# MiraPurkrabek/ProbPose_code

Hardware: AMD Instinct MI355X
Metric: person-crops/sec @ 256x192 bs64 (higher is better)
Workload: dtype f16x3; 1 GPU; ProbPose-small (ViT-S 12x384, 12 heads x 32) bs64 random 256x192 uint8 crops per GPU, flip_test=True, seeded random-init weights: preprocess -> backbone x2 passes -> ProbMapHead (heatmap branch + Sparsemax + 4 towers) -> ProbMap decode -> results in pinned host memory; crops_per_gpu=64, global_batch=64, parallelism=dp1, steps_in_flight=2

## Files before the change

### include/probpose_mi355x.h

```cpp
#ifndef PROBPOSE_MI355X_H_
#define PROBPOSE_MI355X_H_

#include <stddef.h>
#include <stdint.h>

#ifdef __cplusplus
extern "C" {
#endif

#define PP_ABI_VERSION 4


enum {
    PP_OK = 0,
    PP_ERR_INVALID_ARG = -1,
    PP_ERR_UNSUPPORTED = -2,
    PP_ERR_HIP = -3,
    PP_ERR_WORKSPACE = -4
};

#define PP_MAX_RADIUS 9
#define PP_MAX_TAPS (2 * PP_MAX_RADIUS + 1)

int pp_abi_version(void);
const char* pp_last_error(void);
const char* pp_status_string(int status);

int pp_device_cu_count(void);

int pp_stream_create(void** stream_out);
int pp_stream_destroy(void* stream);

int pp_set_option(const char* name, int value);
int pp_get_option(const char* name, int* value);

long long pp_launch_count(const char* kernel);
int pp_reset_launch_counts(void);

typedef struct {
    int prec, n_img, n_tokens, embed, ffn, patch_k, n_keypoints, feat_h, feat_w, heat_h, heat_w, deconv_channels;
} pp_plan_shape;
enum {
    PP_WS_PATCHES = 0,
    PP_WS_X = 1,
    PP_WS_H = 2,
    PP_WS_QKV = 3,
    PP_WS_ATT = 4,
    PP_WS_LN2 = 5,
    PP_WS_FFN = 6,
    PP_WS_FEAT = 7,
    PP_WS_LOGITS = 8,
    PP_WS_DECONV = 9,
    PP_WS_TOWER = 10,
    PP_WS_TOWER_PARTIAL = 11,
    PP_WS_TOWER_POOLED = 12,
    PP_WS_WINOGRAD = 13,
    PP_WS_LN_STATS = 14
};
long long pp_workspace_bytes(int buffer, int index, const pp_plan_shape* shape);

int pp_conv3x3_splitk_slices(int prec, int B, int H, int W, int Cin, int Cout, int groups);

int pp_clock_probe(unsigned long long* out_cycles_ticks, const unsigned long long* stop_flag, unsigned int max_microseconds, void* stream);

int pp_probmap_decode(const float* hm, const float* hm_flip, const int32_t* flip_indices,
                      const double* taps, const int32_t* radius,
                      int B, int K, int H, int W, double in_w, double in_h,
                      float* avg_out, float* conv_out,
                      float* locs, double* keypoints, float* scores, void* stream);

int pp_probmap_head_decode(const float* logits, const float* logits_flip, const int32_t* flip_indices,
                           const double* taps, const int32_t* radius,
                           int B, int K, int H, int W, double in_w, double in_h,
                           float temperature, float normalize,
                           float* avg_out, float* conv_out,
                           float* locs, double* keypoints, float* scores, void* stream);

enum { PP_PREC_BF16 = 0, PP_PREC_F32 = 1, PP_PREC_F16X3 = 2 };
enum { PP_OUT_F32 = 0, PP_OUT_BF16 = 1, PP_OUT_SPLIT = 2 };
enum { PP_ACT_NONE = 0, PP_ACT_GELU = 1, PP_ACT_RELU = 2 };
enum { PP_CONV3X3 = 1, PP_DECONV4X4S2 = 2 };

int pp_gemm(int prec, const void* act, const void* weight, const float* bias, const float* residual,
            int res_mod, void* out, int M, int N, int K, int lda, int ldw, int ldc, int act_fn,
            int out_bf16, int planar_P, void* stream);
int pp_gemm_ws(int prec, const void* act, const void* weight, const float* bias, const float* residual,
               int res_mod, void* out, int M, int N, int K, int lda, int ldw, int ldc, int act_fn,
               int out_bf16, int planar_P, float w_inv_scale, void* stream);

int pp_linear_ln_folded(const void* act, const void* weight, const float* bias, const void* residual, int residual_format,
                        void* out, int out_format, int M, int N, int K, int act_fn, const float* ln_stats,
                        const float* ln_colsum, float ln_eps, float* stats_out, void* stream);
int pp_linear_ln_folded_ws(const void* act, const void* weight, const float* bias, const void* residual, int residual_format,
                           void* out, int out_format, int M, int N, int K, int act_fn, const float* ln_stats,
                           const float* ln_colsum, float ln_eps, float* stats_out, float w_inv_scale, void* stream);
int pp_linear_ln_folded_supported(int M, int N, int K, int with_ln_stats);

int pp_skinny_linear(const void* act, const void* weight, const float* bias, const float* residual, int res_mod, void* out, int out_format,
                     int M, int N, int K, int act_fn, float w_inv_scale, const float* ln_gamma, const float* ln_beta, float ln_eps,
                     void* ln_out, int* ln_counters, void* stream);
int pp_skinny_linear_tile(int M, int N, int K, int with_layernorm);
int pp_skinny_conv1x1_planar(const void* act, const void* weight_padded, const float* bias_padded, float* out, int n_img, int P, int K,
                             int n_valid, float w_inv_scale, void* stream);
int pp_skinny_deconv(const void* act_nhwc, const void* weight, const float* bias, void* out_nhwc, int B, int H, int W, int Cin, int Cout,
                     void* stream);

int pp_gemm_residual_layernorm(int prec, const void* act, const void* weight, const float* bias,
                               const float* residual, int res_mod, float* x_out, const float* gamma,
                               const float* beta, float eps, void* h_out, int h_bf16, int M, int N, int K,
                               int lda, int ldw, void* stream);
int pp_gemm_residual_layernorm_ws(int prec, const void* act, const void* weight, const float* bias,
                               const float* residual, int res_mod, float* x_out, const float* gamma,
                               const float* beta, float eps, void* h_out, int h_bf16, int M, int N, int K,
                               int lda, int ldw, float w_inv_scale, void* stream);

int pp_mlp_residual_layernorm(const void* h_in, const void* w1, const float* b1, const void* w2,
                              const float* b2, const float* residual, float* x_out, const float* gamma,
                              const float* beta, float eps, void* h_out, int M, int E, int F, void* stream);

int pp_proj_mlp_residual_layernorm(const void* attn, const void* wp, const float* bp, const float* residual,
                                   const float* gamma2, const float* beta2, const void* w1, const float* b1,
                                   const void* w2, const float* b2, float* x_out, const float* gamma,
                                   const float* beta, float eps, void* h_out, const void* wqkv, const float* bqkv,
                                   void* qkv_out, int M, int E, int F, void* stream);

int pp_conv_gemm(int prec, int kind, const void* act_nhwc, const void* weight, const float* bias, void* out,
                 int B, int H, int W, int Cin, int Cout, int py, int px, int groups,
                 long long stride_act_g, long long stride_w_g, long long stride_out_g,
                 long long stride_bias_g, int ldc, int act_fn, int out_bf16, void* stream);

int pp_attention(int prec, const void* qkv, void* out, int n_seq, int seq_len, int heads, int head_dim,
                 float scale, void* stream);

int pp_preproc_im2col(int prec, const void* img, int img_is_f32, void* patches, int B, int passes, int H,
                      int W, int patch, int pad, const float* mean_host, const float* std_host,
                      int bgr_to_rgb, void* stream);

int pp_layernorm(const float* x, const float* gamma, const float* beta, void* y, int M, int E, float eps,
                 int out_bf16, void* stream);

int pp_maxpool_relu_nhwc(const void* in, int in_bf16, void* out, int out_bf16, int N, int H, int W, int C,
                         int ph, int pw, void* stream);

int pp_conv3x3_maxpool_relu(int prec, const void* act_nhwc, const void* weight, const float* bias, void* out_pooled,
                            void* scratch_full, int B, int H, int W, int Cin, int Cout, int ph, int pw, int groups,
                            long long stride_act_g, long long stride_w_g, long long stride_bias_g, int fmt, void* stream);

int pp_vit_layer(const void* qkv_in, int seq_len, int heads, float scale, const void* wp, const float* bp,
                 const float* residual, const float* gamma2, const float* beta2, const void* w1, const float* b1,
                 const void* w2, const float* b2, float* x_out, const float* gamma, const float* beta, float eps,
                 void* h_out, const void* wqkv, const float* bqkv, void* qkv_out, int M, int E, int F, void* stream);

long long pp_ffn_split_packed_bytes(int E, int F);
int pp_ffn_split_pack_weights(const void* w1_split, const void* w2_split, void* packed, int E, int F, void* stream);
int pp_ffn_split_residual_layernorm(const void* h_in, const void* w_packed, const float* b1, const float* b2,
                                    const float* residual, float* x_out, const float* gamma, const float* beta,
                                    float eps, void* h_out, int M, int E, int F, void* stream);
int pp_ffn_split_residual_layernorm_ws(const void* h_in, const void* w_packed, const float* b1, const float* b2,
                                       const float* residual, float* x_out, const float* gamma, const float* beta,
                                       float eps, void* h_out, int M, int E, int F, float w1_inv_scale, float w2_inv_scale, void* stream);

int pp_qkv_attention_split(const void* h_in, const void* wqkv, const float* bqkv, void* out, int n_seq, int seq_len, int heads,
                           int head_dim, float scale, void* stream);
int pp_qkv_attention_split_ws(const void* h_in, const void* wqkv, const float* bqkv, void* out, int n_seq, int seq_len, int heads,
                              int head_dim, float scale, float w_inv_scale, void* stream);

int pp_qkv_attention_split_folded(const void* x_centered, const void* wqkv_folded, const float* bqkv_folded, const float* ln_stats, void* out,
                                  int n_seq, int seq_len, int heads, int head_dim, float scale, float w_inv_scale, void* stream);

long long pp_proj_split_packed_bytes(int E);
int pp_proj_split_pack_weights(const void* wp_split, void* packed, int E, void* stream);
int pp_proj_ffn_split_residual_layernorm(const void* att, const void* wproj_packed, const float* bproj,
                                         const float* gamma2, const float* beta2, void* h_scratch, const void* w_packed,
                                         const float* b1, const float* b2, const float* residual, float* x_out,
                                         const float* gamma, const float* beta, float eps, void* h_out, int M, int E,
                                         int F, void* stream);
int pp_proj_ffn_split_residual_layernorm_ws(const void* att, const void* wproj_packed, const float* bproj,
                                            const float* gamma2, const float* beta2, void* h_scratch, const void* w_packed,
                                            const float* b1, const float* b2, const float* residual, float* x_out,
                                            const float* gamma, const float* beta, float eps, void* h_out, int M, int E,
                                            int F, float wp_inv_scale, float w1_inv_scale, float w2_inv_scale, void* stream);

int pp_proj_ffn_split_folded(const void* att, const void* wproj_packed, const float* bproj, const float* gamma2, const float* beta2,
                             void* h_scratch, const void* w_packed, const float* b1, const float* b2, const void* residual,
                             int residual_format, const float* residual_stats, int fold_out, float* x_out, const float* gamma,
                             const float* beta, float eps, void* h_out, float* stats_out, int M, int E, int F, float wp_inv_scale,
                             float w1_inv_scale, float w2_inv_scale, void* stream);

int pp_deconv_head(const void* act_nhwc, const void* weight, const float* bias, const void* head_w, const float* head_b,
                   float* logits_phased, int B, int H, int W, int Cin, int Cout, int K, void* stream);

int pp_deconv_head_split(const void* act_nhwc, const void* weight, const float* bias, const void* head_w_packed,
                         const float* head_b, float* logits_phased, int B, int H, int W, int Cin, int Cout, int K, void* stream);

int pp_probmap_head_decode_phased(const float* logits, const float* logits_flip, const int32_t* flip_indices,
                                  const double* taps, const int32_t* radius, int B, int K, int H, int W, double in_w,
                                  double in_h, float temperature, float normalize, float* avg_out, float* conv_out,
                                  float* locs, double* keypoints, float* scores, void* stream);

#define PP_DECODE_LOGITS 1
#define PP_DECODE_PHASED 2
#define PP_DECODE_SHIFT_HEATMAP 4
int pp_probmap_decode_flags(const float* maps, const float* maps_flip, const int32_t* flip_indices, const double* taps,
                            const int32_t* radius, int B, int K, int H, int W, double in_w, double in_h, float temperature,
                            float normalize, float* avg_out, float* conv_out, float* locs, double* keypoints, float* scores,
                            int flags, void* stream);

int pp_udp_heatmap_decode(const float* maps, const float* maps_flip, const int32_t* flip_indices, int B, int K, int H, int W,
                          double in_w, double in_h, int blur_kernel_size, float* avg_out, float* locs, double* keypoints,
                          float* scores, int flags, void* stream);

int pp_conv3x3_splitk(int prec, const void* act_nhwc, const void* weight, float* partials, int B, int H, int W, int Cin,
                      int Cout, int groups, long long stride_act_g, long long stride_w_g, int ksplit, void* stream);
int pp_sum_maxpool_relu_nhwc(const float* partials, int nsplit, long long split_stride, const float* bias,
                             int images_per_group, void* out, int out_bf16, int N, int H, int W, int C, int ph, int pw,
                             void* stream);

long long pp_winograd_scratch_bytes(int B, int H, int W, int Cin);
int pp_conv3x3_winograd_maxpool_relu(const void* act_nhwc, const void* u_packed, const float* bias, void* v_scratch,
                                     void* out_pooled, int B, int H, int W, int Cin, int Cout, int pool_h, int pool_w, int groups,
                                     void* stream);

int pp_tower_final(const void* feat, int feat_bf16, const float* w, const float* bias,
                   const int32_t* flip_indices, float* out, int B, int passes, int C, int K, float err_div,
                   void* stream);

int pp_extended_oks(const double* gt_kpts, const double* gt_bbox, const double* gt_area, const double* dt_kpts,
                    const double* sigmas, const int* gt_visibilities, int G, int D, int K, int n_vis,
                    double confidence_thr, double padding, int use_area, int original, double* out, void* stream);

int pp_pack_records(const double* keypoints, const float* scores, const float* scalars, double* records, int n, void* stream);

int pp_revert_heatmaps_max(const float* heatmaps, const double* inverse_maps, float* out, int n, int K, int hm_h, int hm_w,
                           int img_h, int img_w, void* stream);

int pp_heatmap_posterior(float* heatmaps, const float* presence, double* scratch, int K, int H, int W, void* stream);

int pp_exoks_cells(const double* gt_kpts, const double* gt_bbox, const double* gt_area, const double* dt_kpts,
                   const double* sigmas, const int* gt_visibilities, const int* cell_gt_off, const int* cell_dt_off,
                   const long long* cell_out_off, int n_cells, int K, int n_vis, double confidence_thr, double padding,
                   int use_area, int original, double* out, void* stream);

int pp_exoks_match(const double* ious, const int* cell_gt_off, const int* cell_dt_off, const long long* cell_iou_off,
                   const unsigned char* gt_ignore, const unsigned char* gt_iscrowd, const double* gt_area,
                   const double* gt_bbox, const double* dt_area, const double* dt_bbox, const double* area_rng,
                   const double* iou_thrs, int n_cells, int max_gt_per_cell, int N_gt, int N_dt, int L, int A, int T,
                   int match_by_bbox, int* dt_match, unsigned char* dt_ignore, int* gt_match,
                   unsigned char* gt_ignore_out, double* sim_sum, int* sim_cnt, void* stream);

int pp_exmap_accumulate(const int* dt_match, const unsigned char* dt_ignore, const unsigned char* gt_ignore,
                        const int* order, const double* dt_score, const double* rec_thrs, int n_cells, int N_gt, int N_dt,
                        int L, int A, int T, int R, int* chunk_scratch, double* precision, double* recall, double* scores,
                        void* stream);

int pp_warp_affine_u8(const void* img_hwc, int img_h, int img_w, int channels, const double* inverse_maps, void* crops_chw,
                      int n, int out_h, int out_w, void* stream);
int pp_warp_affine_u8_batch(const void* const* images, const int* image_hw, int channels, const int* crop_image,
                            const double* inverse_maps, int max_img_h, int max_img_w, void* crops_chw, int n, int out_h,
                            int out_w, void* stream);

long long pp_parea_scratch_bytes(int K, int H, int W);
int pp_parea_thresholds(const float* maps, int K, int H, int W, void* scratch, float* thr, int* draw, void* stream);
int pp_parea_compose(const void* image_rgb, int img_h, int img_w, int pad_left, int pad_top, const float* maps, int K,
                     const float* thr, const int* draw, const int* boxes, int n_boxes, void* canvas_rgb, int canvas_h,
                     int canvas_w, void* stream);
int pp_draw_poses(const void* image_rgb, int img_h, int img_w, const float* keypoints, const float* visible, const int* boxes,
                  int n, int K, const int* skeleton, const void* link_rgb, const void* kpt_rgb, int n_links, double kpt_thr,
                  float radius, float thickness, float alpha, void* out_rgb, void* stream);
int pp_resize_bilinear_u8(const void* src_rgb, int src_h, int src_w, void* dst_rgb, int dst_h, int dst_w, void* stream);

#ifdef __cplusplus
}
#endif
#endif
```

### probpose_code_amd/_lib.py

```python
import ctypes
import os
from ctypes import c_char_p, c_double, c_float, c_int, c_longlong, c_void_p

import torch

_HERE = os.path.dirname(os.path.abspath(__file__))
LIB_NAME = "libprobpose_mi355x.so"
LIB_PATH = os.path.join(_HERE, LIB_NAME)

PP_OK = 0
PP_ERR_INVALID_ARG = -1
PP_ERR_UNSUPPORTED = -2
PP_ERR_HIP = -3
PP_ERR_WORKSPACE = -4
PP_MAX_RADIUS = 9
PP_MAX_TAPS = 2 * PP_MAX_RADIUS + 1


class ProbPoseLibraryError(RuntimeError):

    def __init__(self, fn, status, message):
        super().__init__(f"{fn} failed with {status}: {message}")
        self.status = status


def _load():
    if not os.path.exists(LIB_PATH):
        raise ImportError(
            f"{LIB_PATH} not found. Build it first: `python -c 'import __graft_entry__ as g; g.build()'` "
            "or `make -C probpose_code_amd/csrc`. There is no CPU fallback for the ProbPose hot path."
        )
    return ctypes.CDLL(LIB_PATH)


lib = _load()

_P = c_void_p
SIGNATURES = {
    "pp_abi_version": (c_int, []),
    "pp_last_error": (c_char_p, []),
    "pp_status_string": (c_char_p, [c_int]),
    "pp_device_cu_count": (c_int, []),
    "pp_stream_create": (c_int, [_P]),
    "pp_stream_destroy": (c_int, [_P]),
    "pp_set_option": (c_int, [c_char_p, c_int]),
    "pp_get_option": (c_int, [c_char_p, _P]),
    "pp_launch_count": (c_longlong, [c_char_p]),
    "pp_reset_launch_counts": (c_int, []),
    "pp_workspace_bytes": (c_longlong, [c_int, c_int, _P]),
    "pp_conv3x3_splitk_slices": (c_int, [c_int] * 7),
    "pp_linear_ln_folded": (c_int, [_P, _P, _P, _P, c_int, _P, c_int, c_int, c_int, c_int, c_int, _P, _P, c_float, _P, _P]),
    "pp_linear_ln_folded_ws": (c_int, [_P, _P, _P, _P, c_int, _P, c_int, c_int, c_int, c_int, c_int, _P, _P, c_float, _P, c_float, _P]),
    "pp_linear_ln_folded_supported": (c_int, [c_int] * 4),
    "pp_skinny_linear": (c_int, [_P, _P, _P, _P, c_int, _P, c_int, c_int, c_int, c_int, c_int, c_float, _P, _P, c_float, _P, _P, _P]),
    "pp_skinny_linear_tile": (c_int, [c_int, c_int, c_int, c_int]),
    "pp_skinny_deconv": (c_int, [_P, _P, _P, _P, c_int, c_int, c_int, c_int, c_int, _P]),
    "pp_skinny_conv1x1_planar": (c_int, [_P, _P, _P, _P, c_int, c_int, c_int, c_int, c_float, _P]),
    "pp_clock_probe": (c_int, [_P, _P, ctypes.c_uint, _P]),
    "pp_probmap_decode": (
        c_int,
        [_P, _P, _P, _P, _P, c_int, c_int, c_int, c_int, c_double, c_double, _P, _P, _P, _P, _P, _P],
    ),
    "pp_probmap_head_decode": (
        c_int,
        [_P, _P, _P, _P, _P, c_int, c_int, c_int, c_int, c_double, c_double, c_float, c_float, _P, _P, _P, _P, _P, _P],
    ),
    "pp_probmap_head_decode_phased": (
        c_int,
        [_P, _P, _P, _P, _P, c_int, c_int, c_int, c_int, c_double, c_double, c_float, c_float, _P, _P, _P, _P, _P, _P],
    ),
    "pp_probmap_decode_flags": (
        c_int,
        [_P, _P, _P, _P, _P, c_int, c_int, c_int, c_int, c_double, c_double, c_float, c_float, _P, _P, _P, _P, _P, c_int, _P],
    ),
    "pp_udp_heatmap_decode": (
        c_int, [_P, _P, _P, c_int, c_int, c_int, c_int, c_double, c_double, c_int, _P, _P, _P, _P, c_int, _P]),
    "pp_deconv_head": (c_int, [_P, _P, _P, _P, _P, _P, c_int, c_int, c_int, c_int, c_int, c_int, _P]),
    "pp_deconv_head_split": (c_int, [_P, _P, _P, _P, _P, _P, c_int, c_int, c_int, c_int, c_int, c_int, _P]),
    "pp_gemm": (
        c_int,
        [c_int, _P, _P, _P, _P, c_int, _P, c_int, c_int, c_int, c_int, c_int, c_int, c_int, c_int, c_int, _P],
    ),
    "pp_gemm_ws": (
        c_int,
        [c_int, _P, _P, _P, _P, c_int, _P, c_int, c_int, c_int, c_int, c_int, c_int, c_int, c_int, c_int, c_float, _P],
    ),
    "pp_gemm_residual_layernorm": (
        c_int,
        [c_int, _P, _P, _P, _P, c_int, _P, _P, _P, c_float, _P, c_int, c_int, c_int, c_int, c_int, c_int, _P],
    ),
    "pp_gemm_residual_layernorm_ws": (
        c_int,
        [c_int, _P, _P, _P, _P, c_int, _P, _P, _P, c_float, _P, c_int, c_int, c_int, c_int, c_int, c_int, c_float, _P],
    ),
    "pp_mlp_residual_layernorm": (c_int, [_P, _P, _P, _P, _P, _P, _P, _P, _P, c_float, _P, c_int, c_int, c_int, _P]),
    "pp_proj_mlp_residual_layernorm": (
        c_int, [_P, _P, _P, _P, _P, _P, _P, _P, _P, _P, _P, _P, _P, c_float, _P, _P, _P, _P, c_int, c_int, c_int, _P]),
    "pp_vit_layer": (
        c_int, [_P, c_int, c_int, c_float, _P, _P, _P, _P, _P, _P, _P, _P, _P, _P, _P, _P, c_float, _P, _P, _P, _P, c_int, c_int,
                c_int, _P]),
    "pp_ffn_split_packed_bytes": (c_longlong, [c_int, c_int]),
    "pp_ffn_split_pack_weights": (c_int, [_P, _P, _P, c_int, c_int, _P]),
    "pp_ffn_split_residual_layernorm": (c_int, [_P, _P, _P, _P, _P, _P, _P, _P, c_float, _P, c_int, c_int, c_int, _P]),
    "pp_ffn_split_residual_layernorm_ws": (c_int, [_P, _P, _P, _P, _P, _P, _P, _P, c_float, _P, c_int, c_int, c_int, c_float, c_float, _P]),
    "pp_qkv_attention_split": (c_int, [_P, _P, _P, _P, c_int, c_int, c_int, c_int, c_float, _P]),
    "pp_qkv_attention_split_ws": (c_int, [_P, _P, _P, _P, c_int, c_int, c_int, c_int, c_float, c_float, _P]),
    "pp_qkv_attention_split_folded": (c_int, [_P] * 5 + [c_int] * 4 + [c_float, c_float, _P]),
    "pp_proj_split_packed_bytes": (c_longlong, [c_int]),
    "pp_proj_split_pack_weights": (c_int, [_P, _P, c_int, _P]),
    "pp_proj_ffn_split_residual_layernorm": (
        c_int, [_P, _P, _P, _P, _P, _P, _P, _P, _P, _P, _P, _P, _P, c_float, _P, c_int, c_int, c_int, _P]),
    "pp_proj_ffn_split_residual_layernorm_ws": (
        c_int, [_P, _P, _P, _P, _P, _P, _P, _P, _P, _P, _P, _P, _P, c_float, _P, c_int, c_int, c_int, c_float, c_float, c_float, _P]),
    "pp_proj_ffn_split_folded": (
        c_int, [_P] * 10 + [c_int, _P, c_int, _P, _P, _P, c_float, _P, _P, c_int, c_int, c_int, c_float, c_float, c_float, _P]),
    "pp_conv3x3_splitk": (c_int, [c_int, _P, _P, _P, c_int, c_int, c_int, c_int, c_int, c_int, c_longlong, c_longlong, c_int, _P]),
    "pp_sum_maxpool_relu_nhwc": (c_int, [_P, c_int, c_longlong, _P, c_int, _P, c_int, c_int, c_int, c_int, c_int, c_int, c_int, _P]),
    "pp_warp_affine_u8": (c_int, [_P, c_int, c_int, c_int, _P, _P, c_int, c_int, c_int, _P]),
    "pp_warp_affine_u8_batch": (c_int, [_P, _P, c_int, _P, _P, c_int, c_int, _P, c_int, c_int, c_int, _P]),
    "pp_extended_oks": (
        c_int, [_P, _P, _P, _P, _P, _P, c_int, c_int, c_int, c_int, c_double, c_double, c_int, c_int, _P, _P]),
    "pp_pack_records": (c_int, [_P, _P, _P, _P, c_int, _P]),
    "pp_revert_heatmaps_max": (c_int, [_P, _P, _P] + [c_int] * 6 + [_P]),
    "pp_heatmap_posterior": (c_int, [_P, _P, _P, c_int, c_int, c_int, _P]),
    "pp_exoks_cells": (
        c_int, [_P] * 9 + [c_int, c_int, c_int, c_double, c_double, c_int, c_int, _P, _P]),
    "pp_exoks_match": (
        c_int, [_P] * 12 + [c_int] * 8 + [_P] * 7),
    "pp_exmap_accumulate": (
        c_int, [_P] * 6 + [c_int] * 7 + [_P] * 5),
    "pp_conv_gemm": (
        c_int,
        [c_int, c_int, _P, _P, _P, _P, c_int, c_int, c_int, c_int, c_int, c_int, c_int, c_int,
         c_longlong, c_longlong, c_longlong, c_longlong, c_int, c_int, c_int, _P],
    ),
    "pp_attention": (c_int, [c_int, _P, _P, c_int, c_int, c_int, c_int, c_float, _P]),
    "pp_preproc_im2col": (c_int, [c_int, _P, c_int, _P, c_int, c_int, c_int, c_int, c_int, c_int, _P, _P, c_int, _P]),
    "pp_layernorm": (c_int, [_P, _P, _P, _P, c_int, c_int, c_float, c_int, _P]),
    "pp_maxpool_relu_nhwc": (c_int, [_P, c_int, _P, c_int, c_int, c_int, c_int, c_int, c_int, c_int, _P]),
    "pp_conv3x3_maxpool_relu": (c_int, [c_int, _P, _P, _P, _P, _P] + [c_int] * 8 + [c_longlong] * 3 + [c_int, _P]),
    "pp_winograd_scratch_bytes": (c_longlong, [c_int] * 4),
    "pp_conv3x3_winograd_maxpool_relu": (c_int, [_P] * 5 + [c_int] * 8 + [_P]),
    "pp_tower_final": (c_int, [_P, c_int, _P, _P, _P, _P, c_int, c_int, c_int, c_int, c_float, _P]),
    "pp_parea_scratch_bytes": (c_longlong, [c_int, c_int, c_int]),
    "pp_parea_thresholds": (c_int, [_P, c_int, c_int, c_int, _P, _P, _P, _P]),
    "pp_parea_compose": (c_int, [_P, c_int, c_int, c_int, c_int, _P, c_int, _P, _P, _P, c_int, _P, c_int, c_int, _P]),
    "pp_draw_poses": (
        c_int, [_P, c_int, c_int, _P, _P, _P, c_int, c_int, _P, _P, _P, c_int, c_double, c_float, c_float, c_float, _P, _P]),
    "pp_resize_bilinear_u8": (c_int, [_P, c_int, c_int, _P, c_int, c_int, _P]),
}

for _name, (_res, _args) in SIGNATURES.items():
    _fn = getattr(lib, _name)
    _fn.restype = _res
    _fn.argtypes = _args


class PlanShape(ctypes.Structure):
    _fields_ = [(n, c_int) for n in ("prec", "n_img", "n_tokens", "embed", "ffn", "patch_k", "n_keypoints", "feat_h", "feat_w",
                                     "heat_h", "heat_w", "deconv_channels")]


WS = dict(patches=0, x=1, h=2, qkv=3, att=4, ln2=5, ffn=6, feat=7, logits=8, deconv=9, tower=10, tower_partial=11, tower_pooled=12, winograd=13, ln_stats=14)


def workspace_bytes(buffer: str, shape: "PlanShape", index: int = 0) -> int:
    n = lib.pp_workspace_bytes(WS[buffer], index, ctypes.byref(shape))
    if n < 0:
        raise ProbPoseLibraryError("pp_workspace_bytes", lib.pp_status_string(int(n)).decode(), last_error())
    return int(n)


_option_epoch = 0


_option_first_values = {}


def set_option(name: str, value: int) -> None:
    global _option_epoch
    if name not in _option_first_values:
        v = ctypes.c_int(0)
        if lib.pp_get_option(name.encode(), ctypes.byref(v)) == PP_OK:
            _option_first_values[name] = int(v.value)
    check("pp_set_option", lib.pp_set_option(name.encode(), int(value)))
    _option_epoch += 1


def restore_options() -> None:
    for name, v in list(_option_first_values.items()):
        if get_option(name) != v:
            set_option(name, v)


def option_epoch() -> int:
    return _option_epoch


def launch_count(kernel: str) -> int:
    return int(lib.pp_launch_count(kernel.encode()))


def reset_launch_counts() -> None:
    lib.pp_reset_launch_counts()


def get_option(name: str) -> int:
    v = c_int(0)
    check("pp_get_option", lib.pp_get_option(name.encode(), ctypes.byref(v)))
    return v.value


def _options_from_env() -> None:
    import warnings

    for k, v in os.environ.items():
        if not k.startswith("PP_OPT_"):
            continue
        try:
            set_option(k[len("PP_OPT_"):].lower(), int(v))
        except (ValueError, ProbPoseLibraryError) as exc:
            warnings.warn(f"ignoring {k}={v!r}: {exc}", RuntimeWarning, stacklevel=2)


def last_error() -> str:
    return lib.pp_last_error().decode("utf-8", "replace")


def check(fn_name: str, status: int) -> None:
    if status != PP_OK:
        name = lib.pp_status_string(status).decode()
        raise ProbPoseLibraryError(fn_name, name, last_error())


def ptr(t):
    if t is None:
        return None
    assert t.is_contiguous(), "C ABI takes dense row-major buffers"
    return t.data_ptr()


def stream_ptr(device=None):
    import torch

    return torch.cuda.current_stream(device).cuda_stream


def call(fn_name: str, *args):
    check(fn_name, getattr(lib, fn_name)(*args))


_options_from_env()
```

### probpose_code_amd/csrc/pp_api.hip

```cpp
#include "pp_common.h"

#include <cstring>
#include <mutex>

namespace pp {

static thread_local char g_last_error[512] = "";

void set_error(const char* fmt, ...) {
    va_list ap;
    va_start(ap, fmt);
    vsnprintf(g_last_error, sizeof(g_last_error), fmt, ap);
    va_end(ap);
}

struct Option { const char* name; int value; };
static Option g_options[] = {
    {"panel", 1},
    {"conv_halo", 1},
    {"psplit_nst", 0},
    {"panel_linear_mink", 0},
    {"psplit_bf16_conv", 0},
    {"psplit_tap_inner", 1},
    {"psplit_conv_weight_major", 1},
    {"attn_dma", 1},
    {"conv_pool_split", 1},
    {"decode_wgs_per_cu", 3},
    {"linear_dma", 1},
    {"linear_loop", 1},
    {"psplit_deconv_weight_major", 0},
    {"ffn_pair", 1},
    {"psplit_tail", 1},
    {"wino_order", 8},
    {"ksplit_channels", 1},
    {"qkv_attn_deep", 1},
    {"skinny_tile", 0},
    {"qkv_attn_qsplit", 1},
    {"skinny_xcd_order", 1},
    {"ksplit9_below", 1024},
};

struct LaunchCount {
    char name[48];
    long long n;
};
static LaunchCount g_launches[96];
static int g_n_launches = 0;
static std::mutex g_launch_mutex;

void count_launch(const char* file_or_tag) {
    std::lock_guard<std::mutex> lock(g_launch_mutex);
    const char* base = file_or_tag;
    for (const char* c = file_or_tag; *c; ++c)
        if (*c == '/') base = c + 1;
    for (int i = 0; i < g_n_launches; ++i)
        if (std::strcmp(g_launches[i].name, base) == 0) {
            ++g_launches[i].n;
            return;
        }
    if (g_n_launches < (int)(sizeof(g_launches) / sizeof(g_launches[0]))) {
        std::snprintf(g_launches[g_n_launches].name, sizeof(g_launches[0].name), "%s", base);
        g_launches[g_n_launches++].n = 1;
    }
}

int option(const char* name) {
    for (const Option& o : g_options)
        if (std::strcmp(o.name, name) == 0) return o.value;
    return 0;
}

__global__ void clock_probe_kernel(unsigned long long* out, const unsigned long long* stop, unsigned long long ticks) {
    if (threadIdx.x != 0) return;
    const unsigned long long r0 = __builtin_amdgcn_s_memrealtime();
    const unsigned long long c0 = __builtin_amdgcn_s_memtime();
    unsigned long long r1 = r0;
    for (long long guard = 0; guard < (1ll << 21) && r1 - r0 < ticks; ++guard) {
        if (stop && __hip_atomic_load(stop, __ATOMIC_RELAXED, __HIP_MEMORY_SCOPE_SYSTEM) != 0) break;
        __builtin_amdgcn_s_sleep(127);
        r1 = __builtin_amdgcn_s_memrealtime();
    }
    const unsigned long long c1 = __builtin_amdgcn_s_memtime();
    r1 = __builtin_amdgcn_s_memrealtime();
    __hip_atomic_store(out + 0, c1 - c0, __ATOMIC_RELAXED, __HIP_MEMORY_SCOPE_SYSTEM);
    __hip_atomic_store(out + 1, r1 - r0, __ATOMIC_RELAXED, __HIP_MEMORY_SCOPE_SYSTEM);
}

}

extern "C" {

int pp_set_option(const char* name, int value) {
    using namespace pp;
    PP_REQUIRE(name, PP_ERR_INVALID_ARG, "pp_set_option: NULL name");
    for (Option& o : g_options)
        if (std::strcmp(o.name, name) == 0) {
            o.value = value;
            return PP_OK;
        }
    set_error("pp_set_option: unknown option '%s'", name);
    return PP_ERR_INVALID_ARG;
}

int pp_get_option(const char* name, int* value) {
    using namespace pp;
    PP_REQUIRE(name && value, PP_ERR_INVALID_ARG, "pp_get_option: NULL argument");
    for (const Option& o : g_options)
        if (std::strcmp(o.name, name) == 0) {
            *value = o.value;
            return PP_OK;
        }
    set_error("pp_get_option: unknown option '%s'", name);
    return PP_ERR_INVALID_ARG;
}

long long pp_launch_count(const char* kernel) {
    using namespace pp;
    if (!kernel) {
        set_error("pp_launch_count: NULL name");
        return 0;
    }
    std::lock_guard<std::mutex> lock(g_launch_mutex);
    for (int i = 0; i < g_n_launches; ++i)
        if (std::strcmp(g_launches[i].name, kernel) == 0) return g_launches[i].n;
    return 0;
}

int pp_reset_launch_counts(void) {
    std::lock_guard<std::mutex> lock(pp::g_launch_mutex);
    pp::g_n_launches = 0;
    return PP_OK;
}

long long pp_workspace_bytes(int buffer, int index, const pp_plan_shape* sh) {
    using namespace pp;
    if (!sh || sh->n_img <= 0 || sh->n_tokens <= 0 || sh->embed <= 0 || sh->ffn <= 0 || sh->n_keypoints <= 0 || sh->feat_h <= 0 || sh->feat_w <= 0 ||
        (sh->prec != PP_PREC_BF16 && sh->prec != PP_PREC_F32 && sh->prec != PP_PREC_F16X3)) {
        set_error("pp_workspace_bytes: bad plan shape");
        return PP_ERR_INVALID_ARG;
    }
    const long long esz = sh->prec == PP_PREC_BF16 ? 2 : 4;
    const long long M = (long long)sh->n_img * sh->n_tokens, E = sh->embed;
    auto tower_hw = [&](int j, long long& h, long long& w, long long& ph, long long& pw) {
        h = sh->feat_h;
        w = sh->feat_w;
        for (int i = 0;; ++i) {
            ph = i == 0 ? 4 : 2;
            pw = i == 0 ? 3 : 2;
            if (i == j) return;
            h /= ph;
            w /= pw;
        }
    };
    switch (buffer) {
        case PP_WS_PATCHES: return M * sh->patch_k * esz;
        case PP_WS_X: return M * E * 4;
        case PP_WS_H: case PP_WS_FEAT: case PP_WS_ATT: case PP_WS_LN2: return M * E * esz;
        case PP_WS_QKV: return M * 3 * E * esz;
        case PP_WS_FFN: return M * (long long)sh->ffn * esz;
        case PP_WS_LOGITS: return (long long)sh->n_img * sh->n_keypoints * sh->heat_h * sh->heat_w * 4;
        case PP_WS_DECONV: {
            if (index < 0 || index >= 8 || sh->deconv_channels <= 0) break;
            const long long up = 2ll << index;
            return (long long)sh->n_img * sh->feat_h * up * sh->feat_w * up * sh->deconv_channels * esz;
        }
        case PP_WS_TOWER: case PP_WS_TOWER_PARTIAL: case PP_WS_TOWER_POOLED: {
            if (index < 0 || index > 2) break;
            long long h, w, ph, pw;
            tower_hw(index, h, w, ph, pw);
            if (buffer == PP_WS_TOWER) return 4ll * sh->n_img * h * w * E * esz;
            if (buffer == PP_WS_TOWER_PARTIAL)
                return (long long)pp_conv3x3_splitk_slices(sh->prec, sh->n_img, (int)h, (int)w, sh->embed, sh->embed, 4) * 4 * sh->n_img * h * w * E * 4;
            return 4ll * sh->n_img * (h / ph) * (w / pw) * E * esz;
        }
        case PP_WS_LN_STATS: return E % 96 == 0 ? M * (E / 96) * 8 : 0;
        case PP_WS_WINOGRAD: {
            const long long n = pp_winograd_scratch_bytes(sh->n_img, sh->feat_h, sh->feat_w, sh->embed);
            return n > 0 ? n : 0;
        }
        default: break;
    }
    set_error("pp_workspace_bytes: unknown buffer %d (index %d)", buffer, index);
    return PP_ERR_INVALID_ARG;
}

int pp_conv3x3_splitk_slices(int prec, int B, int H, int W, int Cin, int Cout, int groups) {
    const long long rows = (long long)B * H * W;
    if (prec == PP_PREC_F16X3 && pp::option("panel") && pp::option("ksplit_channels") && pp::option("psplit_tap_inner") >= 1 && Cin % 128 == 0 &&
        Cout % 192 == 0 && ((rows + 255) / 256) * (Cout / 192) * groups * 4 >= 192)
        return 4;
    return rows < pp::option("ksplit9_below") ? 9 : 3;
}

int pp_abi_version(void) { return PP_ABI_VERSION; }

const char* pp_last_error(void) { return pp::g_last_error; }

const char* pp_status_string(int status) {
    switch (status) {
        case PP_OK: return "PP_OK";
        case PP_ERR_INVALID_ARG: return "PP_ERR_INVALID_ARG";
        case PP_ERR_UNSUPPORTED: return "PP_ERR_UNSUPPORTED";
        case PP_ERR_HIP: return "PP_ERR_HIP";
        case PP_ERR_WORKSPACE: return "PP_ERR_WORKSPACE";
        default: return "PP_ERR_UNKNOWN";
    }
}

int pp_clock_probe(unsigned long long* out_cycles_ticks, const unsigned long long* stop_flag, unsigned int max_microseconds, void* stream) {
    using namespace pp;
    PP_REQUIRE(out_cycles_ticks, PP_ERR_INVALID_ARG, "pp_clock_probe: NULL output");
    PP_REQUIRE(max_microseconds <= 5000000u, PP_ERR_INVALID_ARG, "pp_clock_probe: at most 5 s");
    hipLaunchKernelGGL(clock_probe_kernel, dim3(1), dim3(64), 0, (hipStream_t)stream, out_cycles_ticks, stop_flag,
                       (unsigned long long)max_microseconds * 100ull);
    PP_HIP_CHECK(hipGetLastError());
    return PP_OK;
}

int pp_stream_create(void** stream_out) {
    PP_REQUIRE(stream_out != nullptr, PP_ERR_INVALID_ARG, "pp_stream_create: NULL argument");
    hipStream_t s = nullptr;
    PP_HIP_CHECK(hipStreamCreateWithFlags(&s, hipStreamNonBlocking));
    *stream_out = reinterpret_cast<void*>(s);
    return PP_OK;
}

int pp_stream_destroy(void* stream) {
    if (stream == nullptr) return PP_OK;
    PP_HIP_CHECK(hipStreamDestroy(reinterpret_cast<hipStream_t>(stream)));
    return PP_OK;
}

int pp_device_cu_count(void) {
    int dev = 0;
    PP_HIP_CHECK(hipGetDevice(&dev));
    hipDeviceProp_t prop;
    PP_HIP_CHECK(hipGetDeviceProperties(&prop, dev));
    return prop.multiProcessorCount;
}

}
```

### probpose_code_amd/csrc/pp_gemm_ln.hip

```cpp
#include "pp_common.h"
#include "pp_split.h"

namespace pp {

typedef __bf16 bf16x8 __attribute__((ext_vector_type(8)));
typedef __bf16 bf16x4 __attribute__((ext_vector_type(4)));
typedef float f32x4 __attribute__((ext_vector_type(4)));
typedef unsigned int u32x4 __attribute__((ext_vector_type(4)));
typedef __attribute__((address_space(3))) void* lds_ptr_t;

namespace rl {

constexpr int ROW_BYTES = 128;
constexpr int BNH = 384;
template <int BM_, int NH_, int RW_, int CW_, int MINW_>
struct Cfg {
    static constexpr int BM = BM_, NH = NH_, BN = BNH * NH_, RW = RW_, CW = CW_, MINW = MINW_;
    static constexpr int WAVES = RW * CW, THREADS = 64 * WAVES;
    static constexpr int W_TILE = BNH * ROW_BYTES;
    static constexpr int A_TILE = BM * ROW_BYTES;
    static constexpr int STAGE = W_TILE + A_TILE;
    static constexpr int DMA_PER_STAGE = (BNH + BM) / 8;
    static constexpr int DPW = (DMA_PER_STAGE + WAVES - 1) / WAVES;
    static constexpr int RFW = BM / 16 / RW, NFW = BNH / 16 / CW;
    static_assert(RFW * RW * 16 == BM && NFW * CW * 16 == BNH, "wave tiling");
    static constexpr int STAT_BYTES = CW * BM * 4;
    static constexpr int LDS = 2 * STAGE + 2 * STAT_BYTES;
};
typedef Cfg<96, 1, 3, 4, 3> C384;
typedef Cfg<112, 2, 1, 8, 2> C768;
constexpr unsigned OOB_OFFSET = 0x7ffffff0u;

struct Params {
    const void* A;
    const void* W;
    const float* bias;
    const float* residual;
    float* x_out;
    void* h_out;
    const float* gamma;
    const float* beta;
    int M, K, lda, ldw, res_mod, h_bf16;
    unsigned a_bytes, w_bytes;
    float eps;
    float w_s = 1.0f, w_inv = 1.0f;
};

template <typename T>
struct Prec;
template <>
struct Prec<__bf16> {
    static constexpr int BK = 64;
};
template <>
struct Prec<float> {
    static constexpr int BK = 32;
};
template <>
struct Prec<SplitH> {
    static constexpr int BK = 32;
};

__device__ __forceinline__ int swz(int row, int chunk) { return row * ROW_BYTES + ((chunk ^ (row & 7)) << 4); }

__device__ __forceinline__ f32x4 mma(const u32x4& a, const u32x4& b, f32x4 c, __bf16) {
    return __builtin_amdgcn_mfma_f32_16x16x32_bf16(__builtin_bit_cast(bf16x8, a), __builtin_bit_cast(bf16x8, b), c, 0,
                                                   0, 0);
}
__device__ __forceinline__ f32x4 mma(const u32x4& a, const u32x4& b, f32x4 c, float) {
    const f32x4 af = __builtin_bit_cast(f32x4, a), bf = __builtin_bit_cast(f32x4, b);
#pragma unroll
    for (int j = 0; j < 4; ++j) c = __builtin_amdgcn_mfma_f32_16x16x4f32(af[j], bf[j], c, 0, 0, 0);
    return c;
}

template <typename T, typename C>
__global__ __launch_bounds__(C::THREADS, C::MINW) void gemm_res_ln_kernel(const Params p) {
    constexpr int BK = Prec<T>::BK;
    constexpr int ESZ = (int)sizeof(T);
    constexpr int BM = C::BM, BN = C::BN, NH = C::NH, RW = C::RW, CW = C::CW, RFW = C::RFW, NFW = C::NFW, DPW = C::DPW;
    constexpr int STAGE = C::STAGE, W_TILE = C::W_TILE;
    extern __shared__ __attribute__((aligned(16))) char smem[];
    const int tid = threadIdx.x, lane = tid & 63;
    const int wv = __builtin_amdgcn_readfirstlane(tid >> 6);
    const int rw = wv % RW, cw = wv / RW;
    const int f_row = lane & 15, f_kg = lane >> 4;
    const int m0 = blockIdx.x * BM;

    const __amdgpu_buffer_rsrc_t a_rsrc =
        __builtin_amdgcn_make_buffer_rsrc(const_cast<void*>(p.A), 0, p.a_bytes, 0x00020000);
    const __amdgpu_buffer_rsrc_t w_rsrc =
        __builtin_amdgcn_make_buffer_rsrc(const_cast<void*>(p.W), 0, p.w_bytes, 0x00020000);
    const int d_row = lane >> 3;
    const unsigned d_chunk_bytes = (unsigned)(((lane & 7) ^ d_row) << 4);
    unsigned s_voff[DPW];
#pragma unroll
    for (int j = 0; j < DPW; ++j) {
        const int q = wv * DPW + j;
        if (q < BNH / 8) {
            const int n = q * 8 + d_row;
            s_voff[j] = (unsigned)n * (unsigned)(p.ldw * ESZ) + d_chunk_bytes;
        } else {
            const int m = m0 + (q - BNH / 8) * 8 + d_row;
            s_voff[j] = (q < C::DMA_PER_STAGE && m < p.M) ? (unsigned)m * (unsigned)(p.lda * ESZ) + d_chunk_bytes : OOB_OFFSET;
        }
    }
    const unsigned half_bytes = (unsigned)BNH * (unsigned)(p.ldw * ESZ);
    auto stage = [&](int half, int kt, int buf) {
        char* dst = smem + buf * STAGE + wv * DPW * 1024;
        const unsigned kb = (unsigned)(kt * BK * ESZ);
#pragma unroll
        for (int j = 0; j < DPW; ++j) {
            const int q = wv * DPW + j;
            if (q >= C::DMA_PER_STAGE) continue;
            const unsigned vo = s_voff[j] == OOB_OFFSET ? OOB_OFFSET : s_voff[j] + kb;
            if (q < BNH / 8)
                __builtin_amdgcn_raw_ptr_buffer_load_lds(w_rsrc, (lds_ptr_t)(dst + j * 1024), 16, vo + (unsigned)half * half_bytes, 0, 0, 0);
            else
                __builtin_amdgcn_raw_ptr_buffer_load_lds(a_rsrc, (lds_ptr_t)(dst + j * 1024), 16, vo, 0, 0, 0);
        }
    };

    const int nk = p.K / BK;
    const int k_rot = (int)(blockIdx.x >> 3) % nk;
    auto kstep = [&](int i) { const int k = i + k_rot; return k >= nk ? k - nk : k; };
    stage(0, kstep(0), 0);

    const int m_lane = m0 + rw * (16 * RFW) + f_row;
    auto valid = [&](int rf) { return m_lane + rf * 16 < p.M; };
    auto xrow = [&](int rf) { return (size_t)(m_lane + rf * 16) * BN; };
    f32x4 acc[NH][RFW][NFW];
#pragma unroll
    for (int rf = 0; rf < RFW; ++rf) {
        const int m = m_lane + rf * 16;
        const size_t rrow = p.res_mod > 0 ? (size_t)(m % p.res_mod) * BN : xrow(rf);
#pragma unroll
        for (int h = 0; h < NH; ++h)
#pragma unroll
            for (int nf = 0; nf < NFW; ++nf) {
                const int n = h * BNH + cw * (16 * NFW) + nf * 16 + f_kg * 4;
                f32x4 v = {0.f, 0.f, 0.f, 0.f};
                if (p.bias) v = *reinterpret_cast<const f32x4*>(p.bias + n);
                if (p.residual && valid(rf)) v += *reinterpret_cast<const f32x4*>(p.residual + rrow + n);
                acc[h][rf][nf] = v * p.w_s;
            }
    }
    __syncthreads();
#pragma unroll
    for (int h = 0; h < NH; ++h) {
        for (int kt = 0; kt < nk; ++kt) {
            const int buf = (h * nk + kt) & 1;
            if (kt + 1 < nk) stage(h, kstep(kt + 1), buf ^ 1);
            else if (h + 1 < NH) stage(h + 1, kstep(0), buf ^ 1);
            const char* wbase = smem + buf * STAGE;
            const char* abase = wbase + W_TILE;
            if constexpr (__is_same(T, SplitH) && (RFW > NFW)) {
                f16x8 fwh[NFW], fwl[NFW];
#pragma unroll
                for (int nf = 0; nf < NFW; ++nf) {
                    fwh[nf] = *reinterpret_cast<const f16x8*>(wbase + swz(cw * (16 * NFW) + nf * 16 + f_row, f_kg));
                    fwl[nf] = *reinterpret_cast<const f16x8*>(wbase + swz(cw * (16 * NFW) + nf * 16 + f_row, 4 + f_kg));
                }
#pragma unroll
                for (int rf = 0; rf < RFW; ++rf) {
                    const f16x8 fah = *reinterpret_cast<const f16x8*>(abase + swz(rw * (16 * RFW) + rf * 16 + f_row, f_kg));
                    const f16x8 fal = *reinterpret_cast<const f16x8*>(abase + swz(rw * (16 * RFW) + rf * 16 + f_row, 4 + f_kg));
#pragma unroll
                    for (int nf = 0; nf < NFW; ++nf) acc[h][rf][nf] = split_mma(fwh[nf], fwl[nf], fah, fal, acc[h][rf][nf]);
                }
            } else if constexpr (__is_same(T, SplitH)) {
                f16x8 fah[RFW], fal[RFW];
#pragma unroll
                for (int rf = 0; rf < RFW; ++rf) {
                    fah[rf] = *reinterpret_cast<const f16x8*>(abase + swz(rw * (16 * RFW) + rf * 16 + f_row, f_kg));
                    fal[rf] = *reinterpret_cast<const f16x8*>(abase + swz(rw * (16 * RFW) + rf * 16 + f_row, 4 + f_kg));
                }
#pragma unroll
                for (int nf = 0; nf < NFW; ++nf) {
                    const f16x8 fwh = *reinterpret_cast<const f16x8*>(wbase + swz(cw * (16 * NFW) + nf * 16 + f_row, f_kg));
                    const f16x8 fwl = *reinterpret_cast<const f16x8*>(wbase + swz(cw * (16 * NFW) + nf * 16 + f_row, 4 + f_kg));
#pragma unroll
                    for (int rf = 0; rf < RFW; ++rf) acc[h][rf][nf] = split_mma(fwh, fwl, fah[rf], fal[rf], acc[h][rf][nf]);
                }
            } else {
#pragma unroll
                for (int ks = 0; ks < 2; ++ks) {
                    u32x4 fa[RFW];
#pragma unroll
                    for (int rf = 0; rf < RFW; ++rf) fa[rf] = *reinterpret_cast<const u32x4*>(abase + swz(rw * (16 * RFW) + rf * 16 + f_row, ks * 4 + f_kg));
#pragma unroll
                    for (int nf = 0; nf < NFW; ++nf) {
                        const u32x4 fw = *reinterpret_cast<const u32x4*>(wbase + swz(cw * (16 * NFW) + nf * 16 + f_row, ks * 4 + f_kg));
#pragma unroll
                        for (int rf = 0; rf < RFW; ++rf) acc[h][rf][nf] = mma(fw, fa[rf], acc[h][rf][nf], T{});
                    }
                }
            }
            __syncthreads();
        }
    }

#pragma unroll
    for (int h = 0; h < NH; ++h)
#pragma unroll
        for (int rf = 0; rf < RFW; ++rf)
#pragma unroll
            for (int nf = 0; nf < NFW; ++nf) acc[h][rf][nf] *= p.w_inv;
    float* stat = reinterpret_cast<float*>(smem + 2 * STAGE);
    float mean[RFW], rstd[RFW];
#pragma unroll
    for (int rf = 0; rf < RFW; ++rf) {
        float s = 0.f;
#pragma unroll
        for (int h = 0; h < NH; ++h)
#pragma unroll
            for (int nf = 0; nf < NFW; ++nf) {
                const f32x4 v = acc[h][rf][nf];
                s += (v[0] + v[1]) + (v[2] + v[3]);
            }
        s += __shfl_xor(s, 16);
        s += __shfl_xor(s, 32);
        if (f_kg == 0) stat[cw * BM + rw * (16 * RFW) + rf * 16 + f_row] = s;
    }
    __syncthreads();
#pragma unroll
    for (int rf = 0; rf < RFW; ++rf) {
        const int r = rw * (16 * RFW) + rf * 16 + f_row;
        float sm = 0.f;
#pragma unroll
        for (int c = 0; c < CW; ++c) sm += stat[c * BM + r];
        mean[rf] = sm * (1.0f / BN);
        float q = 0.f;
#pragma unroll
        for (int h = 0; h < NH; ++h)
#pragma unroll
            for (int nf = 0; nf < NFW; ++nf)
#pragma unroll
                for (int j = 0; j < 4; ++j) {
                    const float d = acc[h][rf][nf][j] - mean[rf];
                    q = __builtin_fmaf(d, d, q);
                }
        q += __shfl_xor(q, 16);
        q += __shfl_xor(q, 32);
        if (f_kg == 0) stat[(CW + cw) * BM + r] = q;
    }
    __syncthreads();
#pragma unroll
    for (int rf = 0; rf < RFW; ++rf) {
        const int r = rw * (16 * RFW) + rf * 16 + f_row;
        float var = 0.f;
#pragma unroll
        for (int c = 0; c < CW; ++c) var += stat[(CW + c) * BM + r];
        rstd[rf] = 1.0f / sqrtf(var * (1.0f / BN) + p.eps);
    }
#pragma unroll
    for (int h = 0; h < NH; ++h)
#pragma unroll
        for (int nf = 0; nf < NFW; ++nf) {
            const int n = h * BNH + cw * (16 * NFW) + nf * 16 + f_kg * 4;
            const f32x4 g = *reinterpret_cast<const f32x4*>(p.gamma + n), b = *reinterpret_cast<const f32x4*>(p.beta + n);
#pragma unroll
            for (int rf = 0; rf < RFW; ++rf) {
                if (!valid(rf)) continue;
                const f32x4 v = acc[h][rf][nf];
                const size_t off = xrow(rf) + n;
                *reinterpret_cast<f32x4*>(p.x_out + off) = v;
                f32x4 hv;
#pragma unroll
                for (int j = 0; j < 4; ++j) hv[j] = (v[j] - mean[rf]) * rstd[rf] * g[j] + b[j];
                if (p.h_bf16 == 2) {
                    split_store4(p.h_out, off, hv);
                } else if (p.h_bf16) {
                    const bf16x4 ho = {(__bf16)hv[0], (__bf16)hv[1], (__bf16)hv[2], (__bf16)hv[3]};
                    *reinterpret_cast<bf16x4*>(reinterpret_cast<__bf16*>(p.h_out) + off) = ho;
                } else {
                    *reinterpret_cast<f32x4*>(reinterpret_cast<float*>(p.h_out) + off) = hv;
                }
            }
        }
}

template <typename T, typename C>
static int launch(const Params& p, hipStream_t s) {
    auto kern = gemm_res_ln_kernel<T, C>;
    PP_HIP_CHECK(hipFuncSetAttribute(reinterpret_cast<const void*>(kern), hipFuncAttributeMaxDynamicSharedMemorySize, C::LDS));
    hipLaunchKernelGGL(kern, dim3((p.M + C::BM - 1) / C::BM), dim3(C::THREADS), C::LDS, s, p);
    PP_LAUNCH_CHECK();
    return PP_OK;
}

}
}

extern "C" int pp_gemm_residual_layernorm(int prec, const void* act, const void* weight, const float* bias,
                                          const float* residual, int res_mod, float* x_out, const float* gamma,
                                          const float* beta, float eps, void* h_out, int h_bf16, int M, int N, int K,
                                          int lda, int ldw, void* stream) {
    return pp_gemm_residual_layernorm_ws(prec, act, weight, bias, residual, res_mod, x_out, gamma, beta, eps, h_out, h_bf16, M, N, K, lda, ldw, 1.0f,
                                         stream);
}

extern "C" int pp_gemm_residual_layernorm_ws(int prec, const void* act, const void* weight, const float* bias,
                                             const float* residual, int res_mod, float* x_out, const float* gamma,
                                             const float* beta, float eps, void* h_out, int h_bf16, int M, int N, int K,
                                             int lda, int ldw, float w_inv_scale, void* stream) {
    using namespace pp;
    {
        unsigned u;
        __builtin_memcpy(&u, &w_inv_scale, 4);
        PP_REQUIRE((u >> 31) == 0 && (u & 0x007fffffu) == 0 && ((u >> 23) & 0xffu) >= 127 - 40 && ((u >> 23) & 0xffu) <= 127 + 40, PP_ERR_INVALID_ARG,
                   "pp_gemm_residual_layernorm: the weight scale must be a power of two in [2^-40, 2^40]");
        PP_REQUIRE(w_inv_scale == 1.0f || prec == PP_PREC_F16X3, PP_ERR_INVALID_ARG, "pp_gemm_residual_layernorm: weight scales belong to the split-fp16 mode");
    }
    PP_REQUIRE(act && weight && x_out && gamma && beta && h_out, PP_ERR_INVALID_ARG,
               "pp_gemm_residual_layernorm: NULL argument");
    PP_REQUIRE(N == rl::C384::BN || N == rl::C768::BN, PP_ERR_UNSUPPORTED,
               "pp_gemm_residual_layernorm: the fused kernel is built for N = 384 and N = 768");
    PP_REQUIRE(M > 0 && K > 0, PP_ERR_INVALID_ARG, "pp_gemm_residual_layernorm: M and K must be positive");
    const int bk = prec == PP_PREC_BF16 ? 64 : 32;
    const size_t esz = prec == PP_PREC_BF16 ? 2 : 4;
    PP_REQUIRE(prec == PP_PREC_BF16 || prec == PP_PREC_F32 || prec == PP_PREC_F16X3, PP_ERR_INVALID_ARG,
               "pp_gemm_residual_layernorm: unknown precision");
    PP_REQUIRE(h_bf16 == PP_OUT_F32 || h_bf16 == (prec == PP_PREC_BF16 ? PP_OUT_BF16 : (prec == PP_PREC_F16X3 ? PP_OUT_SPLIT : PP_OUT_F32)),
               PP_ERR_UNSUPPORTED, "pp_gemm_residual_layernorm: h_out is fp32 or the operand format of the precision mode");
    PP_REQUIRE(prec != PP_PREC_F16X3 || (lda % 32 == 0 && ldw % 32 == 0), PP_ERR_UNSUPPORTED,
               "pp_gemm_residual_layernorm: split-fp16 operands need row pitches that are multiples of 32 elements");
    PP_REQUIRE(K % bk == 0 && lda % 8 == 0 && ldw % 8 == 0, PP_ERR_UNSUPPORTED,
               "pp_gemm_residual_layernorm: K must be a multiple of the K-tile, lda/ldw multiples of 8");
    const size_t ab = ((size_t)(M - 1) * lda + K) * esz, wb = ((size_t)(N - 1) * ldw + K) * esz;
    PP_REQUIRE(ab < rl::OOB_OFFSET && wb < rl::OOB_OFFSET, PP_ERR_UNSUPPORTED,
               "pp_gemm_residual_layernorm: operands must be smaller than 2 GiB");
    rl::Params p{};
    p.A = act; p.W = weight; p.bias = bias; p.residual = residual; p.x_out = x_out; p.h_out = h_out;
    p.gamma = gamma; p.beta = beta; p.M = M; p.K = K; p.lda = lda; p.ldw = ldw; p.res_mod = res_mod;
    p.h_bf16 = h_bf16; p.a_bytes = (unsigned)ab; p.w_bytes = (unsigned)wb; p.eps = eps;
    p.w_inv = w_inv_scale; p.w_s = 1.0f / w_inv_scale;
    hipStream_t s = reinterpret_cast<hipStream_t>(stream);
    const bool wide = N == rl::C768::BN;
    if (prec == PP_PREC_BF16) return wide ? rl::launch<__bf16, rl::C768>(p, s) : rl::launch<__bf16, rl::C384>(p, s);
    if (prec == PP_PREC_F16X3) return wide ? rl::launch<SplitH, rl::C768>(p, s) : rl::launch<SplitH, rl::C384>(p, s);
    return wide ? rl::launch<float, rl::C768>(p, s) : rl::launch<float, rl::C384>(p, s);
}
```

### probpose_code_amd/engine.py

```python
import math
import os
import warnings
from typing import Dict, Optional, Sequence

import numpy as np
import ctypes

import torch

from . import _lib
from .codecs import oks_kernel_taps
from .weights import PackedWeights, from_split, pack, to_split

PREC = {"bf16": 0, "f32": 1, "f16x3": 2}
_DTYPE = {"bf16": torch.bfloat16, "f32": torch.float32, "f16x3": torch.float32}
_FMT = {"bf16": 1, "f32": 0, "f16x3": 2}
ACT_NONE, ACT_GELU, ACT_RELU = 0, 1, 2
CONV3X3, DECONV = 1, 2


PLAN_DEFAULTS = dict(fuse_mlp=True, fuse_proj=True, fuse_qkv=True, split_k=True, fuse_attn=True, fuse_head=True, fuse_resln=None,
                     fuse_pool=True, fuse_qkv_attn=True, winograd=True, ln_fold=True, small_plan=True, head_two_streams=True)
SMALL_PLAN_ROWS_BELOW = 6912


def plan_from_env() -> Dict[str, object]:
    out: Dict[str, object] = {}
    for k in PLAN_DEFAULTS:
        v = os.environ.get("PP_" + k.upper())
        if v in ("0", "1"):
            out[k] = v == "1"
    return out


class _CapturedGraph:

    def __init__(self, graph, static_in, out, events, side_stream, raw_stream):
        self.graph, self.static_in, self.out, self.events, self.side_stream, self.raw_stream = graph, static_in, out, events, side_stream, raw_stream

    def release(self):
        if self.graph is None and self.raw_stream is None:
            return
        try:
            if torch.cuda.is_available():
                torch.cuda.synchronize()
        except Exception:
            pass
        self.graph = None
        self.out = self.static_in = None
        self.events = []
        self.side_stream = None
        raw, self.raw_stream = self.raw_stream, None
        if raw:
            try:
                _lib.lib.pp_stream_destroy(ctypes.c_void_p(raw))
            except Exception:
                pass

    def __del__(self):
        self.release()


class ProbPoseEngine:
    def __init__(self, state_dict: Dict[str, torch.Tensor], num_heads: int, img_size=(256, 192), patch_size: int = 16,
                 patch_padding: int = 2, mean=(123.675, 116.28, 103.53), std=(58.395, 57.12, 57.375),
                 bgr_to_rgb: bool = True, temperature: float = 0.5, normalize: Optional[float] = 1.0,
                 input_size: Optional[Sequence[int]] = None, ln_eps: float = 1e-6, precision: str = "f16x3",
                 device="cuda", plan: Optional[Dict[str, object]] = None, head_kind: Optional[str] = None,
                 blur_kernel_size: int = 11):
        if precision not in PREC:
            raise ValueError(f"precision must be one of {list(PREC)}, got {precision!r}")
        self.device = torch.device(device)
        if self.device.type != "cuda":
            raise RuntimeError("ProbPoseEngine runs on the MI355X only; there is no CPU fallback")
        pl = dict(PLAN_DEFAULTS)
        pl.update(plan_from_env())
        pl.update(plan or {})
        unknown = set(pl) - set(PLAN_DEFAULTS)
        if unknown:
            raise ValueError(f"unknown launch-plan switch(es) {sorted(unknown)}; known: {sorted(PLAN_DEFAULTS)}")
        self.plan = pl
        self.precision = precision
        self.prec = PREC[precision]
        self.dtype = _DTYPE[precision]
        self.fmt = _FMT[precision]
        self.w: PackedWeights = pack(state_dict, self.dtype, self.device, split=precision == "f16x3", num_heads=int(num_heads), fold_ln=bool(pl["ln_fold"]))
        self.head_kind = self.w.head_kind
        if head_kind is not None and head_kind != self.head_kind:
            raise ValueError(f"head_kind={head_kind!r}, but the state dict holds the weights of a {self.head_kind!r} head "
                             f"({'no ' if self.head_kind == 'heatmap' else ''}scalar-tower keys)")
        if blur_kernel_size % 2 != 1 or not 1 <= blur_kernel_size <= 2 * _lib.PP_MAX_RADIUS + 1:
            raise ValueError(f"blur_kernel_size must be odd and at most {2 * _lib.PP_MAX_RADIUS + 1}, got {blur_kernel_size}")
        self.blur_kernel_size = int(blur_kernel_size)
        self.heads = num_heads
        self.H, self.W = img_size
        self.P, self.pad = patch_size, patch_padding
        self.Hp = (self.H + 2 * self.pad - self.P) // self.P + 1
        self.Wp = (self.W + 2 * self.pad - self.P) // self.P + 1
        self.Np = self.Hp * self.Wp
        assert self.w["pos_embed"].shape[0] == self.Np, "pos_embed does not match img_size / patch grid"
        self.E = self.w.embed_dims
        self.hd = self.E // num_heads
        self.K = self.w.num_keypoints
        self.up = 2 ** len(self.w.deconv_channels)
        self.Hh, self.Wh = self.Hp * self.up, self.Wp * self.up
        self.input_size = tuple(input_size) if input_size is not None else (self.W, self.H)
        self.mean = (np.asarray(mean, np.float32)).copy()
        self.std = (np.asarray(std, np.float32)).copy()
        self.bgr_to_rgb = bool(bgr_to_rgb)
        self.temperature = float(temperature)
        self.normalize = normalize
        self.ln_eps = float(ln_eps)
        if self.head_kind == "probmap":
            taps, radius = oks_kernel_taps(self.K, self.Hh, self.Wh)
            self.taps = torch.from_numpy(taps).to(self.device)
            self.radius = torch.from_numpy(radius).to(self.device)
        self._ws: Dict[tuple, Dict[str, torch.Tensor]] = {}
        self._flip: Dict[tuple, torch.Tensor] = {}
        self._graphs: Dict[tuple, tuple] = {}
        self.max_graphs = 8
        self._tick = 0
        self._graph_tick: Dict[tuple, int] = {}
        self.graph_captures = 0
        self._opt_epoch = _lib.option_epoch()
        self.fuse_mlp, self.fuse_proj, self.fuse_qkv, self.split_k = pl["fuse_mlp"], pl["fuse_proj"], pl["fuse_qkv"], pl["split_k"]
        self.small_plan = bool(precision == "f16x3" and pl["small_plan"])
        self._final_padded = None
        if self.small_plan and self.w.has("final.w") and self.w["final.w"].dim() == 2:
            fw, fb = self.w["final.w"], self.w["final.b"]
            rows = 32 * ((fw.shape[0] + 31) // 32)
            wp = torch.zeros((rows, fw.shape[1]), dtype=fw.dtype, device=fw.device)
            wp[: fw.shape[0]] = fw
            bp = torch.zeros(rows, dtype=torch.float32, device=fb.device)
            bp[: fb.shape[0]] = fb
            self._final_padded = (wp, bp)
        self.small_rows_below = SMALL_PLAN_ROWS_BELOW
        self.fuse_attn, self.fuse_head, self.fuse_pool = pl["fuse_attn"], pl["fuse_head"], pl["fuse_pool"]
        self.fuse_resln = pl["fuse_resln"] is not False
        self._resln_768 = pl["fuse_resln"] is True
        self._ffn_packed: Dict[int, torch.Tensor] = {}
        self._proj_packed: Dict[int, torch.Tensor] = {}
        if precision == "f16x3" and self.fuse_mlp and _lib.lib.pp_ffn_split_packed_bytes(self.E, self.w.ffn_dims) > 0:
            nbytes = _lib.lib.pp_ffn_split_packed_bytes(self.E, self.w.ffn_dims)
            pbytes = _lib.lib.pp_proj_split_packed_bytes(self.E) if self.fuse_proj else -1
            with torch.cuda.device(self.device):
                for i in range(self.w.num_layers):
                    buf = torch.empty(nbytes // 4, dtype=torch.float32, device=self.device)
                    _lib.call("pp_ffn_split_pack_weights", self.w[f"l{i}.fc1.w"].data_ptr(), self.w[f"l{i}.fc2.w"].data_ptr(),
                              buf.data_ptr(), self.E, self.w.ffn_dims, _lib.stream_ptr(self.device))
                    self._ffn_packed[i] = buf
                    if pbytes > 0:
                        pbuf = torch.empty(pbytes // 4, dtype=torch.float32, device=self.device)
                        _lib.call("pp_proj_split_pack_weights", self.w[f"l{i}.proj.w"].data_ptr(), pbuf.data_ptr(), self.E,
                                  _lib.stream_ptr(self.device))
                        self._proj_packed[i] = pbuf
                torch.cuda.synchronize(self.device)
            if not (pl["small_plan"]):
                for i in range(self.w.num_layers):
                    for name in (f"l{i}.fc1.w", f"l{i}.fc2.w") + ((f"l{i}.proj.w",) if i in self._proj_packed else ()):
                        self.w.t.pop(name, None)
        self.fuse_qkv_attn = precision == "f16x3" and pl["fuse_qkv_attn"] and self.Np == 192 and self.hd == 32 and self.E == 384
        self.ln_fold = bool(precision == "f16x3" and pl["ln_fold"] and not self._proj_packed and not self._ffn_packed
                            and self.w.has("l0.fc1.wf") and self.E % 192 == 0 and self.w.ffn_dims % 192 == 0)
        self.ln_fold_fused = bool(precision == "f16x3" and pl["ln_fold"] and self.fuse_qkv_attn and self._proj_packed and self.w.has("l1.qkv.wf")
                                  and (self.w.ffn_dims // 128) % 2 == 0 and self.w.num_layers >= 2)
        if precision == "f16x3":
            if self.fuse_qkv_attn and self._proj_packed:
                self.layer_plan = "two launches per layer (pp_qkv_attention_split + pp_proj_ffn_split_residual_layernorm)"
                if self.ln_fold_fused:
                    self.layer_plan += "; ln1 of layers 1 .. L - 1 folded into the qkv projection (pp_proj_ffn_split_folded -> pp_qkv_attention_split_folded)"
            elif self._proj_packed:
                self.layer_plan = "three launches per layer (pp_gemm qkv + pp_attention + pp_proj_ffn_split_residual_layernorm)"
            else:
                self.layer_plan = "generic (pp_gemm / pp_attention / pp_layernorm per layer)"
                if self.ln_fold:
                    self.layer_plan += ("; from the row count at which the twelve-wave Linear kernel engages: LayerNorm folded into the Linear "
                                        "layers (pp_linear_ln_folded x4 + pp_attention per layer, residual stream in the operand format)")
                if self.hd == 80:
                    self.layer_plan += "; attention at head dim 80: pp_attention_hd80.hip (the q . k contraction zero-padded to 96 on chip)"
                if self._small_at(1):
                    self.layer_plan += (f"; batches of fewer than {SMALL_PLAN_ROWS_BELOW} token rows: the small-batch plan (pp_skinny_linear x4 + "
                                        "pp_attention per layer, LayerNorm in the Linear launches)")
                elif self.small_plan and self.E > 1024:
                    self.layer_plan += f"; no small-batch plan at E = {self.E} (pp_skinny_linear's LayerNorm tail ends at 1024 columns): this plan at every batch size"
            if pl["fuse_qkv_attn"] and not self.fuse_qkv_attn and self.E == 384 and self.hd == 32:
                warnings.warn(
                    f"ProbPoseEngine: {self.Np}-token sequences ({img_size[0]}x{img_size[1]} input) miss the fused qkv + attention kernel, "
                    f"which is built for 192 tokens (256x192); this model runs {self.layer_plan}", RuntimeWarning, stacklevel=2)
        else:
            self.layer_plan = "bf16 / f32 plan"
        self.winograd = (precision == "f16x3" and pl["winograd"] and self.w.has("tower0.wino")
                         and _lib.lib.pp_winograd_scratch_bytes(1, self.Hp, self.Wp, self.E) > 0)
        if self.w.has("tower0.wino") and not self.winograd:
            self.w.t.pop("tower0.wino")
        self._logits_phased = False
        self._head_stream: Optional[torch.cuda.Stream] = None
        self._capture_events: list = []
        self._eager_events: dict = {}
        self.profile: Optional[Dict[str, list]] = None
        self.stage_hook = None
        self.pools = ((4, 3), (2, 2), (2, 2))
        hs, ws_ = self.Hp, self.Wp
        self.tower_hw = []
        for ph, pw_ in self.pools if self.head_kind == "probmap" else ():
            self.tower_hw.append((hs, ws_))
            hs, ws_ = hs // ph, ws_ // pw_
        if self.head_kind == "probmap" and (hs, ws_) != (1, 1):
            raise ValueError(
                f"scalar towers reduce the {self.Hp}x{self.Wp} feature map to {hs}x{ws_}; the reference "
                "reshapes them to (B, 1, K) (probmap_head.py:780-783), which needs 1x1"
            )

    def ksplit(self, nb: int, th: int, tw: int) -> int:
        return int(_lib.lib.pp_conv3x3_splitk_slices(self.prec, int(nb), int(th), int(tw), self.E, self.E, 4))

    def _workspace(self, B: int, passes: int, slot: int = 0) -> Dict[str, torch.Tensor]:
        self._check_options()
        key = (B, passes, slot)
        if key in self._ws:
            return self._ws[key]
        dev, T, f32 = self.device, self.dtype, torch.float32
        nb = B * passes
        M = nb * self.Np
        E, Fd = self.E, self.w.ffn_dims
        dc = self.w.deconv_channels
        shape = _lib.PlanShape(prec=self.prec, n_img=nb, n_tokens=self.Np, embed=E, ffn=Fd, patch_k=3 * self.P * self.P, n_keypoints=self.K,
                               feat_h=self.Hp, feat_w=self.Wp, heat_h=self.Hh, heat_w=self.Wh, deconv_channels=dc[0] if dc else 0)

        def buf(which, dims, dt=T, index=0):
            nbytes = _lib.workspace_bytes(which, shape, index)
            t = torch.empty(nbytes, dtype=torch.uint8, device=dev).view(dt)
            assert t.numel() == math.prod(dims), (which, index, nbytes, dims)
            return t.view(*dims)

        e = lambda *s, dt=T: torch.empty(s, dtype=dt, device=dev)
        small = self._small_at(M)
        fused_layer = self.precision == "f16x3" and self.fuse_qkv_attn and bool(self._proj_packed) and not small
        ws = dict(
            patches=buf("patches", (M, 3 * self.P * self.P)), x=buf("x", (M, E), f32), h=buf("h", (M, E)),
            feat=buf("feat", (M, E)), logits=buf("logits", (nb, self.K, self.Hh * self.Wh), f32),
            qkv=None if (fused_layer or (small and self.fuse_qkv_attn)) else buf("qkv", (M, 3 * E)),
            qkv2=None if (fused_layer or small) else buf("qkv", (M, 3 * E)),
            f=None if ((fused_layer or self._ffn_packed) and not small) else buf("ffn", (M, Fd)),
            att=buf("att", (M, E)) if (self.fuse_qkv_attn or small) else None,
            hs=buf("ln2", (M, E)) if (self._proj_packed or small) else None,
            ln_count=torch.zeros((M + 31) // 32, dtype=torch.int32, device=dev) if small else None,
            xs=buf("h", (M, E)) if self._ln_fold_at(M) else None,
            lnst=buf("ln_stats", (M, E // 96, 2), f32) if self._ln_fold_at(M) else None,
            rowst=e(M, 2, dt=f32) if self.ln_fold_fused else None,
            scalars=e(4, B, self.K, dt=f32) if self.head_kind == "probmap" else torch.zeros((4, B, self.K), dtype=f32, device=dev),
            locs=e(B, self.K, 2, dt=f32),
            keypoints=e(B, self.K, 2, dt=torch.float64), scores=e(B, self.K, dt=f32),
            heatmaps=e(B, self.K, self.Hh, self.Wh, dt=f32),
        )
        hh, ww = self.Hp, self.Wp
        for j, c in enumerate(dc):
            hh, ww = hh * 2, ww * 2
            if c == dc[0]:
                ws[f"d{j}"] = buf("deconv", (nb, hh, ww, c), index=j)
            else:
                ws[f"d{j}"] = e(nb, hh, ww, c)
        if self.winograd:
            nbytes = _lib.workspace_bytes("winograd", shape)
            ws["wino"] = torch.empty(nbytes, dtype=torch.uint8, device=dev) if 0 < nbytes < 0x7FFFFFF0 else None
        for j, (th, tw) in enumerate(self.tower_hw):
            ph, pw_ = self.pools[j]
            ws[f"t{j}"] = buf("tower", (4, nb, th, tw, E), index=j)
            if nb * th * tw * 4 < 128 * 128:
                ks = self.ksplit(nb, th, tw)
                ws[f"tp{j}"] = buf("tower_partial", (ks, 4, nb, th, tw, E), f32, index=j)
            ws[f"p{j}"] = buf("tower_pooled", (4, nb, th // ph, tw // pw_, E), index=j)
        self._ws[key] = ws
        return ws

    def _small_at(self, M: int) -> bool:
        return bool(self.small_plan and M < self.small_rows_below and self.E % 64 == 0 and self.w.ffn_dims % 64 == 0 and self.E <= 1024
                    and self.w.has("l0.fc1.w") and self.w.has("l0.proj.w") and (3 * self.P * self.P) % 64 == 0)

    def _ln_fold_at(self, M: int) -> bool:
        return (self.ln_fold and _lib.get_option("linear_dma") != 0
                and _lib.lib.pp_linear_ln_folded_supported(int(M), self.E, self.E, 1) == 2
                and _lib.lib.pp_linear_ln_folded_supported(int(M), self.E, self.w.ffn_dims, 0) == 2)

    def _check_options(self) -> None:
        if _lib.option_epoch() != self._opt_epoch:
            self._opt_epoch = _lib.option_epoch()
            self._ws.clear()
            self._graphs.clear()
            self._graph_tick.clear()

    def _flip_indices(self, flip_indices) -> torch.Tensor:
        key = tuple(int(i) for i in flip_indices)
        if key not in self._flip:
            assert len(key) == self.K
            self._flip[key] = torch.tensor(key, dtype=torch.int32, device=self.device)
        return self._flip[key]

    def _call(self, tag: str, fn: str, *args):
        if self.profile is None:
            _lib.call(fn, *args)
            return
        a, b = torch.cuda.Event(enable_timing=True), torch.cuda.Event(enable_timing=True)
        a.record()
        _lib.call(fn, *args)
        b.record()
        self.profile.setdefault(tag, []).append((a, b))

    def _gemm(self, st, a, w, bias, out, M, N, K, act=ACT_NONE, residual=None, res_mod=0, out_bf16=None, planar=0,
              ldc=None, winv: float = 1.0):
        ob = self.fmt if out_bf16 is None else out_bf16
        self._call("gemm_bf16out" if ob else "gemm_f32out", "pp_gemm_ws", self.prec, a.data_ptr(), w.data_ptr(), _lib.ptr(bias), _lib.ptr(residual),
                   res_mod, out.data_ptr(), M, N, K, K, K, N if ldc is None else ldc, act, ob, planar, float(winv), st)

    def backbone(self, imgs_u8: torch.Tensor, passes: int, ws, st) -> torch.Tensor:
        B = imgs_u8.shape[0]
        M = B * passes * self.Np
        E, Fd, w = self.E, self.w.ffn_dims, self.w
        ob = self.fmt
        self._call("im2col", "pp_preproc_im2col", self.prec, imgs_u8.data_ptr(), int(imgs_u8.dtype == torch.float32),
                  ws["patches"].data_ptr(), B, passes, self.H, self.W, self.P, self.pad, self.mean.ctypes.data,
                  self.std.ctypes.data, int(self.bgr_to_rgb), st)
        Kp = 3 * self.P * self.P
        scale = self.hd ** -0.5
        fused = self.fuse_resln and (E == 384 or (E == 768 and self._resln_768))
        L = w.num_layers

        def res_ln(a, wk, bk, K, gamma, beta, h_out, residual=None, res_mod=0, winv=1.0):
            residual = ws["x"] if residual is None else residual
            if fused:
                self._call("gemm_res_ln", "pp_gemm_residual_layernorm_ws", self.prec, a.data_ptr(), wk.data_ptr(),
                           bk.data_ptr(), residual.data_ptr(), res_mod, ws["x"].data_ptr(), gamma.data_ptr(),
                           beta.data_ptr(), self.ln_eps, h_out.data_ptr(), ob, M, E, K, K, K, float(winv), st)
            else:
                self._gemm(st, a, wk, bk, ws["x"], M, E, K, residual=residual, res_mod=res_mod, out_bf16=0, winv=winv)
                self._call("layernorm", "pp_layernorm", ws["x"].data_ptr(), gamma.data_ptr(), beta.data_ptr(),
                           h_out.data_ptr(), M, E, self.ln_eps, ob, st)

        if self._small_at(M):
            return self._layers_small(ws, st, B * passes, M)
        res_ln(ws["patches"], w["patch_w"], w["patch_b"], Kp, w["l0.ln1.w"], w["l0.ln1.b"], ws["h"],
               residual=w["pos_embed"], res_mod=self.Np)
        if self._ln_fold_at(M):
            return self._layers_ln_folded(ws, st, B * passes, M)
        qkv_done = False
        one_launch = (fused and E == 384 and self.precision == "bf16" and Fd % 128 == 0 and self.fuse_mlp and self.fuse_proj and self.fuse_attn
                      and self.Np == 192 and self.hd == 32)
        qcur, qnext = ws["qkv"], ws["qkv2"]
        att = ws["att"] if self.fuse_qkv_attn else ws["h"]
        for i in range(L):
            if not qkv_done and not self.fuse_qkv_attn:
                self._gemm(st, ws["h"], w[f"l{i}.qkv.w"], w[f"l{i}.qkv.b"], qcur, M, 3 * E, E, winv=w.inv(f"l{i}.qkv.w"))
            if self.stage_hook is not None:
                self.stage_hook("embed" if i == 0 else f"layer{i - 1}")
            if one_launch:
                last = i + 1 == L
                gn, bn = (w["ln_f.w"], w["ln_f.b"]) if last else (w[f"l{i + 1}.ln1.w"], w[f"l{i + 1}.ln1.b"])
                nq = None if (last or not self.fuse_qkv) else (w[f"l{i + 1}.qkv.w"], w[f"l{i + 1}.qkv.b"])
                h_next = ws["feat"] if last else ws["h"]
                self._call("vit_layer", "pp_vit_layer", qcur.data_ptr(), self.Np, self.heads, scale, w[f"l{i}.proj.w"].data_ptr(),
                           w[f"l{i}.proj.b"].data_ptr(), ws["x"].data_ptr(), w[f"l{i}.ln2.w"].data_ptr(),
                           w[f"l{i}.ln2.b"].data_ptr(), w[f"l{i}.fc1.w"].data_ptr(), w[f"l{i}.fc1.b"].data_ptr(),
                           w[f"l{i}.fc2.w"].data_ptr(), w[f"l{i}.fc2.b"].data_ptr(), ws["x"].data_ptr(), gn.data_ptr(),
                           bn.data_ptr(), self.ln_eps, None if nq else h_next.data_ptr(), nq[0].data_ptr() if nq else None,
                           nq[1].data_ptr() if nq else None, qnext.data_ptr() if nq else None, M, E, Fd, st)
                qkv_done = nq is not None
                qcur, qnext = qnext, qcur
                continue
            qkv_done = False
            fold = self.ln_fold_fused
            if self.fuse_qkv_attn and fold and i >= 1:
                self._call("qkv_attention", "pp_qkv_attention_split_folded", ws["h"].data_ptr(), w[f"l{i}.qkv.wf"].data_ptr(), w[f"l{i}.qkv.bf"].data_ptr(),
                           ws["rowst"].data_ptr(), att.data_ptr(), B * passes, self.Np, self.heads, self.hd, scale, w.inv(f"l{i}.qkv.wf"), st)
            elif self.fuse_qkv_attn:
                self._call("qkv_attention", "pp_qkv_attention_split_ws", ws["h"].data_ptr(), w[f"l{i}.qkv.w"].data_ptr(),
                           w[f"l{i}.qkv.b"].data_ptr(), att.data_ptr(), B * passes, self.Np, self.heads, self.hd, scale, w.inv(f"l{i}.qkv.w"), st)
            else:
                self._call("attention", "pp_attention", self.prec, qcur.data_ptr(), ws["h"].data_ptr(), B * passes,
                           self.Np, self.heads, self.hd, scale, st)
            last = i + 1 == L
            gn, bn = (w["ln_f.w"], w["ln_f.b"]) if last else (w[f"l{i + 1}.ln1.w"], w[f"l{i + 1}.ln1.b"])
            h_next = ws["feat"] if last else ws["h"]
            fuse_ffn = fused and E == 384 and self.precision == "bf16" and Fd % 128 == 0 and self.fuse_mlp
            if fuse_ffn and self.fuse_proj:
                nq = None if (last or not self.fuse_qkv) else (w[f"l{i + 1}.qkv.w"], w[f"l{i + 1}.qkv.b"])
                self._call("proj_mlp_res_ln", "pp_proj_mlp_residual_layernorm", ws["h"].data_ptr(),
                           w[f"l{i}.proj.w"].data_ptr(), w[f"l{i}.proj.b"].data_ptr(), ws["x"].data_ptr(),
                           w[f"l{i}.ln2.w"].data_ptr(), w[f"l{i}.ln2.b"].data_ptr(), w[f"l{i}.fc1.w"].data_ptr(),
                           w[f"l{i}.fc1.b"].data_ptr(), w[f"l{i}.fc2.w"].data_ptr(), w[f"l{i}.fc2.b"].data_ptr(),
                           ws["x"].data_ptr(), gn.data_ptr(), bn.data_ptr(), self.ln_eps,
                           None if nq else h_next.data_ptr(), nq[0].data_ptr() if nq else None,
                           nq[1].data_ptr() if nq else None, qcur.data_ptr() if nq else None, M, E, Fd, st)
                qkv_done = nq is not None
                continue
            if i in self._proj_packed and self.fuse_qkv_attn and fold:
                res, res_fmt = (ws["x"], 0) if i == 0 else (ws["h"], 2)
                self._call("proj_ffn_split", "pp_proj_ffn_split_folded", att.data_ptr(), self._proj_packed[i].data_ptr(), w[f"l{i}.proj.b"].data_ptr(),
                           w[f"l{i}.ln2.w"].data_ptr(), w[f"l{i}.ln2.b"].data_ptr(), ws["hs"].data_ptr(), self._ffn_packed[i].data_ptr(),
                           w[f"l{i}.fc1.b"].data_ptr(), w[f"l{i}.fc2.b"].data_ptr(), res.data_ptr(), res_fmt, None if i == 0 else ws["rowst"].data_ptr(),
                           0 if last else 1, ws["x"].data_ptr() if last else None, gn.data_ptr() if last else None, bn.data_ptr() if last else None,
                           self.ln_eps, h_next.data_ptr(), None if last else ws["rowst"].data_ptr(), M, E, Fd, w.inv(f"l{i}.proj.w"),
                           w.inv(f"l{i}.fc1.w"), w.inv(f"l{i}.fc2.w"), st)
                continue
            if i in self._proj_packed:
                self._call("proj_ffn_split", "pp_proj_ffn_split_residual_layernorm_ws", att.data_ptr(), self._proj_packed[i].data_ptr(),
                           w[f"l{i}.proj.b"].data_ptr(), w[f"l{i}.ln2.w"].data_ptr(), w[f"l{i}.ln2.b"].data_ptr(), ws["hs"].data_ptr(),
                           self._ffn_packed[i].data_ptr(), w[f"l{i}.fc1.b"].data_ptr(), w[f"l{i}.fc2.b"].data_ptr(),
                           ws["x"].data_ptr(), ws["x"].data_ptr(), gn.data_ptr(), bn.data_ptr(), self.ln_eps, h_next.data_ptr(),
                           M, E, Fd, w.inv(f"l{i}.proj.w"), w.inv(f"l{i}.fc1.w"), w.inv(f"l{i}.fc2.w"), st)
                continue
            res_ln(att, w[f"l{i}.proj.w"], w[f"l{i}.proj.b"], E, w[f"l{i}.ln2.w"], w[f"l{i}.ln2.b"], ws["h"], winv=w.inv(f"l{i}.proj.w"))
            if i in self._ffn_packed:
                self._call("ffn_split", "pp_ffn_split_residual_layernorm_ws", ws["h"].data_ptr(), self._ffn_packed[i].data_ptr(),
                           w[f"l{i}.fc1.b"].data_ptr(), w[f"l{i}.fc2.b"].data_ptr(), ws["x"].data_ptr(), ws["x"].data_ptr(),
                           gn.data_ptr(), bn.data_ptr(), self.ln_eps, h_next.data_ptr(), M, E, Fd, w.inv(f"l{i}.fc1.w"), w.inv(f"l{i}.fc2.w"), st)
            elif fuse_ffn:
                self._call("mlp_res_ln", "pp_mlp_residual_layernorm", ws["h"].data_ptr(), w[f"l{i}.fc1.w"].data_ptr(),
                           w[f"l{i}.fc1.b"].data_ptr(), w[f"l{i}.fc2.w"].data_ptr(), w[f"l{i}.fc2.b"].data_ptr(),
                           ws["x"].data_ptr(), ws["x"].data_ptr(), gn.data_ptr(), bn.data_ptr(), self.ln_eps,
                           h_next.data_ptr(), M, E, Fd, st)
            else:
                self._gemm(st, ws["h"], w[f"l{i}.fc1.w"], w[f"l{i}.fc1.b"], ws["f"], M, Fd, E, act=ACT_GELU, winv=w.inv(f"l{i}.fc1.w"))
                res_ln(ws["f"], w[f"l{i}.fc2.w"], w[f"l{i}.fc2.b"], Fd, gn, bn, h_next, winv=w.inv(f"l{i}.fc2.w"))
        return ws["feat"]

    def _layers_small(self, ws, st, nb: int, M: int) -> torch.Tensor:
        E, Fd, w, L = self.E, self.w.ffn_dims, self.w, self.w.num_layers
        F32, SPLIT = 0, 2
        scale = self.hd ** -0.5
        cnt = ws["ln_count"]

        def lin(a, wname, bias, out, N, K, act=ACT_NONE, residual=None, res_mod=0, out_fmt=SPLIT, ln=None):
            g, b, h_out = ln if ln is not None else (None, None, None)
            self._call("skinny_linear", "pp_skinny_linear", a.data_ptr(), w[wname].data_ptr(), _lib.ptr(bias), _lib.ptr(residual), res_mod,
                       out.data_ptr(), out_fmt, M, N, K, act, w.inv(wname), _lib.ptr(g), _lib.ptr(b), self.ln_eps, _lib.ptr(h_out),
                       cnt.data_ptr() if ln is not None else None, st)

        lin(ws["patches"], "patch_w", w["patch_b"], ws["x"], E, 3 * self.P * self.P, residual=w["pos_embed"], res_mod=self.Np, out_fmt=F32,
            ln=(w["l0.ln1.w"], w["l0.ln1.b"], ws["h"]))
        for i in range(L):
            if self.fuse_qkv_attn:
                self._call("qkv_attention", "pp_qkv_attention_split_ws", ws["h"].data_ptr(), w[f"l{i}.qkv.w"].data_ptr(), w[f"l{i}.qkv.b"].data_ptr(),
                           ws["att"].data_ptr(), nb, self.Np, self.heads, self.hd, scale, w.inv(f"l{i}.qkv.w"), st)
            else:
                lin(ws["h"], f"l{i}.qkv.w", w[f"l{i}.qkv.b"], ws["qkv"], 3 * E, E)
                self._call("attention", "pp_attention", self.prec, ws["qkv"].data_ptr(), ws["att"].data_ptr(), nb, self.Np, self.heads, self.hd, scale, st)
            if self.stage_hook is not None:
                self.stage_hook("embed" if i == 0 else f"layer{i - 1}")
            lin(ws["att"], f"l{i}.proj.w", w[f"l{i}.proj.b"], ws["x"], E, E, residual=ws["x"], out_fmt=F32,
                ln=(w[f"l{i}.ln2.w"], w[f"l{i}.ln2.b"], ws["hs"]))
            lin(ws["hs"], f"l{i}.fc1.w", w[f"l{i}.fc1.b"], ws["f"], Fd, E, act=ACT_GELU)
            last = i + 1 == L
            gn, bn = (w["ln_f.w"], w["ln_f.b"]) if last else (w[f"l{i + 1}.ln1.w"], w[f"l{i + 1}.ln1.b"])
            lin(ws["f"], f"l{i}.fc2.w", w[f"l{i}.fc2.b"], ws["x"], E, Fd, residual=ws["x"], out_fmt=F32, ln=(gn, bn, ws["feat"] if last else ws["h"]))
        return ws["feat"]

    def _layers_ln_folded(self, ws, st, nb: int, M: int) -> torch.Tensor:
        E, Fd, w, L = self.E, self.w.ffn_dims, self.w, self.w.num_layers
        F32, SPLIT = 0, 2
        xs, stt, scale = ws["xs"], ws["lnst"], self.hd ** -0.5

        def lin(a, wname, bias, out, N, K, act=ACT_NONE, residual=None, res_fmt=F32, out_fmt=SPLIT, ln=None, stats_out=None):
            self._call("linear_fold", "pp_linear_ln_folded_ws", a.data_ptr(), w[wname].data_ptr(), bias.data_ptr(), _lib.ptr(residual), res_fmt,
                       out.data_ptr(), out_fmt, M, N, K, act, stt.data_ptr() if ln is not None else None, _lib.ptr(ln), self.ln_eps,
                       stt.data_ptr() if stats_out else None, w.inv(wname), st)

        for i in range(L):
            if i == 0:
                lin(ws["h"], "l0.qkv.w", w["l0.qkv.b"], ws["qkv"], 3 * E, E)
            else:
                lin(xs, f"l{i}.qkv.wf", w[f"l{i}.qkv.bf"], ws["qkv"], 3 * E, E, ln=w[f"l{i}.qkv.cf"])
            if self.stage_hook is not None:
                self.stage_hook("embed" if i == 0 else f"layer{i - 1}")
            self._call("attention", "pp_attention", self.prec, ws["qkv"].data_ptr(), ws["h"].data_ptr(), nb, self.Np, self.heads, self.hd, scale, st)
            lin(ws["h"], f"l{i}.proj.w", w[f"l{i}.proj.b"], xs, E, E, residual=ws["x"] if i == 0 else xs, res_fmt=F32 if i == 0 else SPLIT,
                stats_out=True)
            lin(xs, f"l{i}.fc1.wf", w[f"l{i}.fc1.bf"], ws["f"], Fd, E, act=ACT_GELU, ln=w[f"l{i}.fc1.cf"])
            last = i + 1 == L
            lin(ws["f"], f"l{i}.fc2.w", w[f"l{i}.fc2.b"], ws["x"] if last else xs, E, Fd, residual=xs, res_fmt=SPLIT,
                out_fmt=F32 if last else SPLIT, stats_out=not last)
        self._call("layernorm", "pp_layernorm", ws["x"].data_ptr(), w["ln_f.w"].data_ptr(), w["ln_f.b"].data_ptr(), ws["feat"].data_ptr(), M, E,
                   self.ln_eps, self.fmt, st)
        return ws["feat"]

    def heatmap_logits(self, feat: torch.Tensor, nb: int, ws, st) -> torch.Tensor:
        w = self.w
        ob = self.fmt
        src, cin, hh, ww = feat, self.E, self.Hp, self.Wp
        self._logits_phased = False
        nd = len(w.deconv_channels)
        for j, cout in enumerate(w.deconv_channels):
            dst = ws[f"d{j}"]
            wj = w[f"deconv{j}.w"]
            if (j == nd - 1 and self.fuse_head and ob == 1 and cout == 256 and w.has("final.w_pad") and cin % 32 == 0
                    and ww % 4 == 0 and self.K <= 28):
                self._call("deconv_head", "pp_deconv_head", src.data_ptr(), wj.data_ptr(), w[f"deconv{j}.b"].data_ptr(),
                           w["final.w_pad"].data_ptr(), w["final.b"].data_ptr(), ws["logits"].data_ptr(), nb, hh, ww, cin, cout,
                           self.K, st)
                self._logits_phased = True
                return ws["logits"]
            if (j == nd - 1 and self.fuse_head and ob == 2 and cout == 256 and w.has("final.w_head") and cin % 32 == 0
                    and ww % 4 == 0 and self.K <= 28 and nb * hh * ww * 4 >= 192 * 192):
                self._call("deconv_head", "pp_deconv_head_split", src.data_ptr(), wj.data_ptr(), w[f"deconv{j}.b"].data_ptr(),
                           w["final.w_head"].data_ptr(), w["final.b"].data_ptr(), ws["logits"].data_ptr(), nb, hh, ww, cin, cout,
                           self.K, st)
                self._logits_phased = True
                return ws["logits"]
            if ob == 2 and self._small_at(nb * self.Np) and nb * hh * ww <= 1536 and cin % 32 == 0 and cout % 32 == 0:
                self._call("deconv", "pp_skinny_deconv", src.data_ptr(), wj.data_ptr(), w[f"deconv{j}.b"].data_ptr(), dst.data_ptr(), nb, hh, ww, cin,
                           cout, st)
                src, cin, hh, ww = dst, cout, hh * 2, ww * 2
                continue
            self._call("deconv", "pp_conv_gemm", self.prec, DECONV, src.data_ptr(), wj.data_ptr(),
                       w[f"deconv{j}.b"].data_ptr(), dst.data_ptr(), nb, hh, ww, cin, cout, -1, -1, 1, 0, 0, 0, 0, cout,
                       ACT_RELU, ob, st)
            src, cin, hh, ww = dst, cout, hh * 2, ww * 2
        P = hh * ww
        if ob == 2 and self._small_at(nb * self.Np) and cin % 64 == 0 and self._final_padded is not None:
            wp, bp = self._final_padded
            self._call("final_conv", "pp_skinny_conv1x1_planar", src.data_ptr(), wp.data_ptr(), bp.data_ptr(), ws["logits"].data_ptr(), nb, P, cin, self.K,
                       w.inv("final.w"), st)
            return ws["logits"]
        self._gemm(st, src, w["final.w"], w["final.b"], ws["logits"], nb * P, self.K, cin, planar=P, out_bf16=0)
        return ws["logits"]

    def towers(self, feat: torch.Tensor, B: int, passes: int, flip_indices, ws, st) -> torch.Tensor:
        w, E = self.w, self.E
        nb = B * passes
        ob = self.fmt
        src, stride_src = feat, 0
        for j, (th, tw) in enumerate(self.tower_hw):
            ph, pw_ = self.pools[j]
            out = ws[f"t{j}"]
            rows = nb * th * tw
            if self.split_k and f"tp{j}" in ws:
                part = ws[f"tp{j}"]
                ks = part.shape[0]
                self._call("conv3x3_splitk", "pp_conv3x3_splitk", self.prec, src.data_ptr(), w[f"tower{j}.w"].data_ptr(),
                           part.data_ptr(), nb, th, tw, E, E, 4, stride_src, E * 9 * E, ks, st)
                self._call("maxpool", "pp_sum_maxpool_relu_nhwc", part.data_ptr(), ks, 4 * rows * E, w[f"tower{j}.b"].data_ptr(),
                           nb, ws[f"p{j}"].data_ptr(), ob, 4 * nb, th, tw, E, ph, pw_, st)
                src = ws[f"p{j}"]
                stride_src = nb * (th // ph) * (tw // pw_) * E
                continue
            if j == 0 and self.winograd and ws.get("wino") is not None and stride_src == 0 and (ph, pw_) == (4, 3):
                self._call("conv3x3", "pp_conv3x3_winograd_maxpool_relu", src.data_ptr(), w["tower0.wino"].data_ptr(), w["tower0.b"].data_ptr(),
                           ws["wino"].data_ptr(), ws["p0"].data_ptr(), nb, th, tw, E, E, ph, pw_, 4, st)
            elif self.fuse_pool:
                self._call("conv3x3", "pp_conv3x3_maxpool_relu", self.prec, src.data_ptr(), w[f"tower{j}.w"].data_ptr(),
                           w[f"tower{j}.b"].data_ptr(), ws[f"p{j}"].data_ptr(), out.data_ptr(), nb, th, tw, E, E, ph, pw_, 4,
                           stride_src, E * 9 * E, E, ob, st)
            else:
                self._call("conv3x3", "pp_conv_gemm", self.prec, CONV3X3, src.data_ptr(), w[f"tower{j}.w"].data_ptr(),
                           w[f"tower{j}.b"].data_ptr(), out.data_ptr(), nb, th, tw, E, E, 0, 0, 4, stride_src,
                           E * 9 * E, nb * th * tw * E, E, E, ACT_NONE, ob, st)
                self._call("maxpool", "pp_maxpool_relu_nhwc", out.data_ptr(), ob, ws[f"p{j}"].data_ptr(), ob, 4 * nb, th, tw, E, ph,
                           pw_, st)
            src = ws[f"p{j}"]
            stride_src = nb * (th // ph) * (tw // pw_) * E
        fi = self._flip_indices(flip_indices) if passes == 2 else None
        self._call("tower_final", "pp_tower_final", src.data_ptr(), ob, w["tower_out.w"].data_ptr(), w["tower_out.b"].data_ptr(),
                  _lib.ptr(fi), ws["scalars"].data_ptr(), B, passes, E, self.K, 1.0, st)
        return ws["scalars"]

    def _check_imgs(self, imgs: torch.Tensor):
        assert imgs.dim() == 4 and imgs.is_cuda, "expects a (B,3,H,W) tensor on the GPU"
        assert imgs.dtype in (torch.uint8, torch.float32), "crops are uint8 (raw) or float32 (already preprocessed)"
        assert tuple(imgs.shape[1:]) == (3, self.H, self.W), f"crop shape {tuple(imgs.shape)} != (B,3,{self.H},{self.W})"

    @torch.no_grad()
    def run_backbone(self, imgs: torch.Tensor, flip_test: bool, slot: int = 0) -> torch.Tensor:
        self._check_imgs(imgs)
        imgs = imgs.contiguous()
        B, passes = imgs.shape[0], 2 if flip_test else 1
        ws = self._workspace(B, passes, slot)
        with torch.cuda.device(self.device):
            feat = self.backbone(imgs, passes, ws, _lib.stream_ptr(self.device))
        return feat.view(B * passes, self.Hp, self.Wp, self.E)

    def export_features(self, feat: torch.Tensor) -> torch.Tensor:
        return from_split(feat) if self.precision == "f16x3" else feat.clone()

    def import_features(self, x_nhwc: torch.Tensor) -> torch.Tensor:
        if self.precision == "f16x3":
            return to_split(x_nhwc.float().contiguous())
        if x_nhwc.dtype != self.dtype or not x_nhwc.is_contiguous():
            x_nhwc = x_nhwc.to(self.dtype).contiguous()
        return x_nhwc

    @torch.no_grad()
    def run_head(self, feat_nhwc: torch.Tensor, flip_test: bool, flip_indices=None,
                 return_heatmaps: bool = False, slot: int = 0, shift_heatmap: bool = False) -> Dict[str, torch.Tensor]:
        passes = 2 if flip_test else 1
        nb = feat_nhwc.shape[0]
        assert nb % passes == 0 and tuple(feat_nhwc.shape[1:]) == (self.Hp, self.Wp, self.E)
        assert feat_nhwc.dtype == self.dtype and feat_nhwc.is_contiguous() and feat_nhwc.is_cuda
        if flip_test and flip_indices is None:
            raise ValueError("flip_test needs flip_indices (dataset meta)")
        B = nb // passes
        ws = self._workspace(B, passes, slot)
        if self.head_kind == "heatmap":
            with torch.cuda.device(self.device):
                st = _lib.stream_ptr(self.device)
                logits = self.heatmap_logits(feat_nhwc, nb, ws, st)
                fi = self._flip_indices(flip_indices) if flip_test else None
                lf = logits[B:] if flip_test else None
                flags = (2 if self._logits_phased else 0) | (4 if (shift_heatmap and flip_test) else 0)
                self._call("head_decode", "pp_udp_heatmap_decode", logits.data_ptr(), _lib.ptr(lf), _lib.ptr(fi), B, self.K, self.Hh, self.Wh,
                           float(self.input_size[0]), float(self.input_size[1]), self.blur_kernel_size,
                           ws["heatmaps"].data_ptr() if return_heatmaps else None, ws["locs"].data_ptr(), ws["keypoints"].data_ptr(),
                           ws["scores"].data_ptr(), flags, st)
            out = dict(keypoints=ws["keypoints"], scores=ws["scores"], locs=ws["locs"], scalars=ws["scalars"])
            if return_heatmaps:
                out["heatmaps"] = ws["heatmaps"]
            return out
        two = self.plan["head_two_streams"] and self._small_at(nb * self.Np)
        with torch.cuda.device(self.device):
            cur = torch.cuda.current_stream(self.device)
            scalars = None
            if two:
                if self._head_stream is None:
                    self._head_stream = torch.cuda.Stream(device=self.device)
                self._fork_join(cur, self._head_stream)
                with torch.cuda.stream(self._head_stream):
                    scalars = self.towers(feat_nhwc, B, passes, flip_indices, ws, _lib.stream_ptr(self.device))
            st = _lib.stream_ptr(self.device)
            logits = self.heatmap_logits(feat_nhwc, nb, ws, st)
            fi = self._flip_indices(flip_indices) if flip_test else None
            lf = logits[B:] if flip_test else None
            flags = 1 | (2 if self._logits_phased else 0) | (4 if (shift_heatmap and flip_test) else 0)
            self._call("head_decode", "pp_probmap_decode_flags", logits.data_ptr(), _lib.ptr(lf), _lib.ptr(fi), self.taps.data_ptr(),
                      self.radius.data_ptr(), B, self.K, self.Hh, self.Wh, float(self.input_size[0]),
                      float(self.input_size[1]), self.temperature, -1.0 if self.normalize is None else float(self.normalize),
                      ws["heatmaps"].data_ptr() if return_heatmaps else None, None, ws["locs"].data_ptr(),
                      ws["keypoints"].data_ptr(), ws["scores"].data_ptr(), flags, st)
            if two:
                self._fork_join(self._head_stream, cur)
            else:
                scalars = self.towers(feat_nhwc, B, passes, flip_indices, ws, st)
        out = dict(keypoints=ws["keypoints"], scores=ws["scores"], locs=ws["locs"], scalars=scalars)
        if return_heatmaps:
            out["heatmaps"] = ws["heatmaps"]
        return out

    @torch.no_grad()
    def forward(self, imgs: torch.Tensor, flip_test: bool = True, flip_indices=None, return_heatmaps: bool = False,
                return_features: bool = False, slot: int = 0, shift_heatmap: bool = False) -> Dict[str, torch.Tensor]:
        self._tick += 1
        feat = self.run_backbone(imgs, flip_test, slot)
        out = self.run_head(feat, flip_test, flip_indices, return_heatmaps, slot, shift_heatmap)
        if return_features:
            out["features"] = feat
        return out

    def _fork_join(self, producer: torch.cuda.Stream, consumer: torch.cuda.Stream) -> None:
        if torch.cuda.is_current_stream_capturing():
            ev = torch.cuda.Event()
            self._capture_events.append(ev)
        else:
            key = (producer.cuda_stream, consumer.cuda_stream)
            ev = self._eager_events.get(key)
            if ev is None:
                ev = self._eager_events[key] = torch.cuda.Event()
        ev.record(producer)
        consumer.wait_event(ev)

    def capture(self, B: int, flip_test: bool = True, flip_indices=None, return_heatmaps: bool = False, slot: int = 0,
                shift_heatmap: bool = False):
        self._check_options()
        key = (B, flip_test, tuple(flip_indices) if flip_indices is not None else None, return_heatmaps, bool(shift_heatmap), slot)
        if key in self._graphs:
            self._graphs[key] = self._graphs.pop(key)
            return self._graphs[key].static_in
        while len(self._graphs) >= max(1, int(self.max_graphs)):
            old_key = next(iter(self._graphs))
            torch.cuda.synchronize(self.device)
            self._graphs.pop(old_key).release()
            self._graph_tick.pop(old_key, None)
            passes_old = 2 if old_key[1] else 1
            if not any(k[0] == old_key[0] and k[-1] == old_key[-1] and (2 if k[1] else 1) == passes_old for k in self._graphs):
                self._ws.pop((old_key[0], passes_old, old_key[-1]), None)
        static_in = torch.zeros((B, 3, self.H, self.W), dtype=torch.uint8, device=self.device)
        raw = ctypes.c_void_p()
        _lib.check("pp_stream_create", _lib.lib.pp_stream_create(ctypes.byref(raw)))
        eager_head_stream, self._head_stream = self._head_stream, torch.cuda.ExternalStream(raw.value, device=self.device)
        side = torch.cuda.Stream(device=self.device)
        try:
            side.wait_stream(torch.cuda.current_stream(self.device))
            with torch.cuda.stream(side):
                for _ in range(2):
                    self.forward(static_in, flip_test, flip_indices, return_heatmaps, slot=slot, shift_heatmap=shift_heatmap)
            torch.cuda.current_stream(self.device).wait_stream(side)
            side.synchronize()
            graph = torch.cuda.CUDAGraph()
            self._capture_events = []
            with torch.cuda.graph(graph):
                out = self.forward(static_in, flip_test, flip_indices, return_heatmaps, slot=slot, shift_heatmap=shift_heatmap)
            self._graphs[key] = _CapturedGraph(graph, static_in, out, self._capture_events, self._head_stream, raw.value)
            raw = None
        finally:
            self._capture_events = []
            self._head_stream = eager_head_stream
            if raw is not None and raw.value:
                torch.cuda.synchronize(self.device)
                _lib.lib.pp_stream_destroy(raw)
        self._graph_tick[key] = self._tick
        self.graph_captures += 1
        return static_in

    @staticmethod
    def _graph_key(B, flip_test, flip_indices, return_heatmaps, shift_heatmap, slot):
        return (B, flip_test, tuple(flip_indices) if flip_indices is not None else None, return_heatmaps, bool(shift_heatmap), slot)

    def has_graph(self, B: int, flip_test: bool = True, flip_indices=None, return_heatmaps: bool = False, slot: int = 0,
                  shift_heatmap: bool = False) -> bool:
        self._check_options()
        return self._graph_key(B, flip_test, flip_indices, return_heatmaps, shift_heatmap, slot) in self._graphs

    def capture_would_thrash(self) -> bool:
        if len(self._graphs) < max(1, int(self.max_graphs)):
            return False
        victim = next(iter(self._graphs))
        return self._tick - self._graph_tick.get(victim, 0) <= 64 * max(1, int(self.max_graphs))

    def forward_graph(self, imgs: torch.Tensor, flip_test: bool = True, flip_indices=None,
                      return_heatmaps: bool = False, slot: int = 0, shift_heatmap: bool = False) -> Dict[str, torch.Tensor]:
        B = imgs.shape[0]
        static_in = self.capture(B, flip_test, flip_indices, return_heatmaps, slot, shift_heatmap)
        key = self._graph_key(B, flip_test, flip_indices, return_heatmaps, shift_heatmap, slot)
        graph, out = self._graphs[key].graph, self._graphs[key].out
        self._tick += 1
        self._graph_tick[key] = self._tick
        if imgs.data_ptr() != static_in.data_ptr():
            static_in.copy_(imgs, non_blocking=True)
        graph.replay()
        return out


F16X3_MAX_OPERAND = 65504.0
F16X3_FULL_PRECISION_MIN = 0.125
F16X3_FOLD_MEAN_OVER_STD = 30.0


@torch.no_grad()
def domain_report(state_dict: Dict[str, torch.Tensor], crops_u8: torch.Tensor, num_heads: int, img_size=(256, 192), device="cuda",
                  **engine_kw) -> Dict[str, object]:
    eng = ProbPoseEngine(state_dict, num_heads, img_size=img_size, precision="f32", device=device, **engine_kw)
    rows: list = []
    crops_u8 = crops_u8.to(eng.device)
    B = crops_u8.shape[0]
    ws = eng._workspace(B, 1, 0)

    def stat(name, t):
        t = t.float()
        return {name + "_absmax": float(t.abs().max())}

    def hook(stage):
        torch.cuda.synchronize(eng.device)
        x = ws["x"].float()
        sd_ = x.std(dim=1, unbiased=False).clamp_min(1e-12)
        r = dict(stage=stage, residual_absmax=float(x.abs().max()), residual_mean_over_std=float((x.mean(dim=1).abs() / sd_).max()))
        r.update(stat("ln_out", ws["h"]))
        r.update(stat("qkv", ws["qkv"]))
        if ws.get("f") is not None and stage != "embed":
            r.update(stat("ffn_hidden", ws["f"]))
        rows.append(r)

    eng.stage_hook = hook
    out = eng.forward(crops_u8, False, None)
    torch.cuda.synchronize(eng.device)
    eng.stage_hook = None
    feat_abs = float(ws["feat"].float().abs().max())
    worst = max(max(v for k, v in r.items() if k.endswith("_absmax")) for r in rows)
    worst = max(worst, feat_abs)
    ratio = max(r["residual_mean_over_std"] for r in rows[1:]) if len(rows) > 1 else 0.0
    finite = bool(torch.isfinite(out["keypoints"]).all())
    ok = finite and worst <= F16X3_MAX_OPERAND / 2 and ratio <= F16X3_FOLD_MEAN_OVER_STD
    advice = "inside the f16x3 domain"
    if not finite or worst > F16X3_MAX_OPERAND / 2:
        advice = (f"an operand reaches {worst:.3g} (limit 65504, a factor 2 kept in hand): run precision='f32', or rescale the layer that "
                  "produces it")
    elif ratio > F16X3_FOLD_MEAN_OVER_STD:
        advice = (f"token rows reach |mean| / std = {ratio:.1f}: the folded LayerNorm loses ~log2 of that in bits - build the model with "
                  "plan=dict(ln_fold=False) (LayerNorm applied before the split, no cancellation)")
    return dict(layers=rows, features_absmax=feat_abs, max_operand=worst, max_mean_over_std=ratio, ok=ok, advice=advice)
```

Baseline: 14980 crops/s.

## Fuse uint8 preprocessing and im2col into patch-embed GEMM with residual layernorm

Adds a patch_embed_ln kernel that reads uint8 crops directly, normalizes them and forms the split-fp16 patch operand inside the GEMM+residual+LayerNorm kernel. This removes the separate im2col launch and its patches buffer round-trip through HBM. The shared GEMM body moves into an included header so the existing kernel and the new one use the same code. The cost is extra per-tile preprocessing work inside the GEMM loader, and the fused path is limited to f16x3 precision, 384-wide embeddings and patch 16.

```diff
diff --git a/include/probpose_mi355x.h b/include/probpose_mi355x.h
--- a/include/probpose_mi355x.h
+++ b/include/probpose_mi355x.h
@@ -136,6 +136,13 @@
                       int W, int patch, int pad, const float* mean_host, const float* std_host,
                       int bgr_to_rgb, void* stream);
 
+int pp_patch_embed_layernorm_supported(int prec, int img_is_f32, int M, int N, int K, int H, int W, int patch, int pad);
+int pp_patch_embed_layernorm_ws(const void* img, int img_is_f32, int B, int passes, int H, int W, int patch, int pad,
+                                const float* mean_host, const float* std_host, int bgr_to_rgb, int prec, const void* weight,
+                                const float* bias, const float* residual, int res_mod, float* x_out, const float* gamma,
+                                const float* beta, float eps, void* h_out, int h_bf16, int M, int N, int K, int ldw,
+                                float w_inv_scale, void* stream);
+
 int pp_layernorm(const float* x, const float* gamma, const float* beta, void* y, int M, int E, float eps,
                  int out_bf16, void* stream);
 
diff --git a/probpose_code_amd/_lib.py b/probpose_code_amd/_lib.py
--- a/probpose_code_amd/_lib.py
+++ b/probpose_code_amd/_lib.py
@@ -136,6 +136,12 @@
     ),
     "pp_attention": (c_int, [c_int, _P, _P, c_int, c_int, c_int, c_int, c_float, _P]),
     "pp_preproc_im2col": (c_int, [c_int, _P, c_int, _P, c_int, c_int, c_int, c_int, c_int, c_int, _P, _P, c_int, _P]),
+    "pp_patch_embed_layernorm_supported": (c_int, [c_int] * 9),
+    "pp_patch_embed_layernorm_ws": (
+        c_int,
+        [_P, c_int, c_int, c_int, c_int, c_int, c_int, c_int, _P, _P, c_int, c_int, _P, _P, _P, c_int, _P, _P, _P, c_float, _P, c_int, c_int, c_int,
+         c_int, c_int, c_float, _P],
+    ),
     "pp_layernorm": (c_int, [_P, _P, _P, _P, c_int, c_int, c_float, c_int, _P]),
     "pp_maxpool_relu_nhwc": (c_int, [_P, c_int, _P, c_int, c_int, c_int, c_int, c_int, c_int, c_int, _P]),
     "pp_conv3x3_maxpool_relu": (c_int, [c_int, _P, _P, _P, _P, _P] + [c_int] * 8 + [c_longlong] * 3 + [c_int, _P]),
diff --git a/probpose_code_amd/csrc/pp_api.hip b/probpose_code_amd/csrc/pp_api.hip
--- a/probpose_code_amd/csrc/pp_api.hip
+++ b/probpose_code_amd/csrc/pp_api.hip
@@ -37,6 +37,7 @@
     {"skinny_tile", 0},
     {"qkv_attn_qsplit", 1},
     {"skinny_xcd_order", 1},
+    {"patch_embed_fused", 1},
     {"ksplit9_below", 1024},
 };
 
diff --git a/probpose_code_amd/csrc/pp_gemm_ln.hip b/probpose_code_amd/csrc/pp_gemm_ln.hip
--- a/probpose_code_amd/csrc/pp_gemm_ln.hip
+++ b/probpose_code_amd/csrc/pp_gemm_ln.hip
@@ -1,3 +1,5 @@
+#include <type_traits>
+
 #include "pp_common.h"
 #include "pp_split.h"
 
@@ -46,6 +48,14 @@
     float w_s = 1.0f, w_inv = 1.0f;
 };
 
+struct PatchParams : Params {
+    const unsigned char* img;
+    unsigned img_bytes;
+    int B, IH, IW, Wp, Np, pad, bgr_to_rgb;
+    float m0, m1, m2, s0, s1, s2;
+};
+constexpr int PE_ITEMS = 2 * 96;
+
 template <typename T>
 struct Prec;
 template <>
@@ -74,210 +84,29 @@
     return c;
 }
 
+template <int PE, typename P>
+__device__ __forceinline__ const P& pe_params(const P& p) { return p; }
+
 template <typename T, typename C>
 __global__ __launch_bounds__(C::THREADS, C::MINW) void gemm_res_ln_kernel(const Params p) {
-    constexpr int BK = Prec<T>::BK;
-    constexpr int ESZ = (int)sizeof(T);
-    constexpr int BM = C::BM, BN = C::BN, NH = C::NH, RW = C::RW, CW = C::CW, RFW = C::RFW, NFW = C::NFW, DPW = C::DPW;
-    constexpr int STAGE = C::STAGE, W_TILE = C::W_TILE;
-    extern __shared__ __attribute__((aligned(16))) char smem[];
-    const int tid = threadIdx.x, lane = tid & 63;
-    const int wv = __builtin_amdgcn_readfirstlane(tid >> 6);
-    const int rw = wv % RW, cw = wv / RW;
-    const int f_row = lane & 15, f_kg = lane >> 4;
-    const int m0 = blockIdx.x * BM;
-
-    const __amdgpu_buffer_rsrc_t a_rsrc =
-        __builtin_amdgcn_make_buffer_rsrc(const_cast<void*>(p.A), 0, p.a_bytes, 0x00020000);
-    const __amdgpu_buffer_rsrc_t w_rsrc =
-        __builtin_amdgcn_make_buffer_rsrc(const_cast<void*>(p.W), 0, p.w_bytes, 0x00020000);
-    const int d_row = lane >> 3;
-    const unsigned d_chunk_bytes = (unsigned)(((lane & 7) ^ d_row) << 4);
-    unsigned s_voff[DPW];
-#pragma unroll
-    for (int j = 0; j < DPW; ++j) {
-        const int q = wv * DPW + j;
-        if (q < BNH / 8) {
-            const int n = q * 8 + d_row;
-            s_voff[j] = (unsigned)n * (unsigned)(p.ldw * ESZ) + d_chunk_bytes;
-        } else {
-            const int m = m0 + (q - BNH / 8) * 8 + d_row;
-            s_voff[j] = (q < C::DMA_PER_STAGE && m < p.M) ? (unsigned)m * (unsigned)(p.lda * ESZ) + d_chunk_bytes : OOB_OFFSET;
-        }
-    }
-    const unsigned half_bytes = (unsigned)BNH * (unsigned)(p.ldw * ESZ);
-    auto stage = [&](int half, int kt, int buf) {
-        char* dst = smem + buf * STAGE + wv * DPW * 1024;
-        const unsigned kb = (unsigned)(kt * BK * ESZ);
-#pragma unroll
-        for (int j = 0; j < DPW; ++j) {
-            const int q = wv * DPW + j;
-            if (q >= C::DMA_PER_STAGE) continue;
-            const unsigned vo = s_voff[j] == OOB_OFFSET ? OOB_OFFSET : s_voff[j] + kb;
-            if (q < BNH / 8)
-                __builtin_amdgcn_raw_ptr_buffer_load_lds(w_rsrc, (lds_ptr_t)(dst + j * 1024), 16, vo + (unsigned)half * half_bytes, 0, 0, 0);
-            else
-                __builtin_amdgcn_raw_ptr_buffer_load_lds(a_rsrc, (lds_ptr_t)(dst + j * 1024), 16, vo, 0, 0, 0);
-        }
-    };
-
-    const int nk = p.K / BK;
-    const int k_rot = (int)(blockIdx.x >> 3) % nk;
-    auto kstep = [&](int i) { const int k = i + k_rot; return k >= nk ? k - nk : k; };
-    stage(0, kstep(0), 0);
-
-    const int m_lane = m0 + rw * (16 * RFW) + f_row;
-    auto valid = [&](int rf) { return m_lane + rf * 16 < p.M; };
-    auto xrow = [&](int rf) { return (size_t)(m_lane + rf * 16) * BN; };
-    f32x4 acc[NH][RFW][NFW];
-#pragma unroll
-    for (int rf = 0; rf < RFW; ++rf) {
-        const int m = m_lane + rf * 16;
-        const size_t rrow = p.res_mod > 0 ? (size_t)(m % p.res_mod) * BN : xrow(rf);
-#pragma unroll
-        for (int h = 0; h < NH; ++h)
-#pragma unroll
-            for (int nf = 0; nf < NFW; ++nf) {
-                const int n = h * BNH + cw * (16 * NFW) + nf * 16 + f_kg * 4;
-                f32x4 v = {0.f, 0.f, 0.f, 0.f};
-                if (p.bias) v = *reinterpret_cast<const f32x4*>(p.bias + n);
-                if (p.residual && valid(rf)) v += *reinterpret_cast<const f32x4*>(p.residual + rrow + n);
-                acc[h][rf][nf] = v * p.w_s;
-            }
-    }
-    __syncthreads();
-#pragma unroll
-    for (int h = 0; h < NH; ++h) {
-        for (int kt = 0; kt < nk; ++kt) {
-            const int buf = (h * nk + kt) & 1;
-            if (kt + 1 < nk) stage(h, kstep(kt + 1), buf ^ 1);
-            else if (h + 1 < NH) stage(h + 1, kstep(0), buf ^ 1);
-            const char* wbase = smem + buf * STAGE;
-            const char* abase = wbase + W_TILE;
-            if constexpr (__is_same(T, SplitH) && (RFW > NFW)) {
-                f16x8 fwh[NFW], fwl[NFW];
-#pragma unroll
-                for (int nf = 0; nf < NFW; ++nf) {
-                    fwh[nf] = *reinterpret_cast<const f16x8*>(wbase + swz(cw * (16 * NFW) + nf * 16 + f_row, f_kg));
-                    fwl[nf] = *reinterpret_cast<const f16x8*>(wbase + swz(cw * (16 * NFW) + nf * 16 + f_row, 4 + f_kg));
-                }
-#pragma unroll
-                for (int rf = 0; rf < RFW; ++rf) {
-                    const f16x8 fah = *reinterpret_cast<const f16x8*>(abase + swz(rw * (16 * RFW) + rf * 16 + f_row, f_kg));
-                    const f16x8 fal = *reinterpret_cast<const f16x8*>(abase + swz(rw * (16 * RFW) + rf * 16 + f_row, 4 + f_kg));
-#pragma unroll
-                    for (int nf = 0; nf < NFW; ++nf) acc[h][rf][nf] = split_mma(fwh[nf], fwl[nf], fah, fal, acc[h][rf][nf]);
-                }
-            } else if constexpr (__is_same(T, SplitH)) {
-                f16x8 fah[RFW], fal[RFW];
-#pragma unroll
-                for (int rf = 0; rf < RFW; ++rf) {
-                    fah[rf] = *reinterpret_cast<const f16x8*>(abase + swz(rw * (16 * RFW) + rf * 16 + f_row, f_kg));
-                    fal[rf] = *reinterpret_cast<const f16x8*>(abase + swz(rw * (16 * RFW) + rf * 16 + f_row, 4 + f_kg));
-                }
-#pragma unroll
-                for (int nf = 0; nf < NFW; ++nf) {
-                    const f16x8 fwh = *reinterpret_cast<const f16x8*>(wbase + swz(cw * (16 * NFW) + nf * 16 + f_row, f_kg));
-                    const f16x8 fwl = *reinterpret_cast<const f16x8*>(wbase + swz(cw * (16 * NFW) + nf * 16 + f_row, 4 + f_kg));
-#pragma unroll
-                    for (int rf = 0; rf < RFW; ++rf) acc[h][rf][nf] = split_mma(fwh, fwl, fah[rf], fal[rf], acc[h][rf][nf]);
-                }
-            } else {
-#pragma unroll
-                for (int ks = 0; ks < 2; ++ks) {
-                    u32x4 fa[RFW];
-#pragma unroll
-                    for (int rf = 0; rf < RFW; ++rf) fa[rf] = *reinterpret_cast<const u32x4*>(abase + swz(rw * (16 * RFW) + rf * 16 + f_row, ks * 4 + f_kg));
-#pragma unroll
-                    for (int nf = 0; nf < NFW; ++nf) {
-                        const u32x4 fw = *reinterpret_cast<const u32x4*>(wbase + swz(cw * (16 * NFW) + nf * 16 + f_row, ks * 4 + f_kg));
-#pragma unroll
-                        for (int rf = 0; rf < RFW; ++rf) acc[h][rf][nf] = mma(fw, fa[rf], acc[h][rf][nf], T{});
-                    }
-                }
-            }
-            __syncthreads();
-        }
-    }
-
-#pragma unroll
-    for (int h = 0; h < NH; ++h)
-#pragma unroll
-        for (int rf = 0; rf < RFW; ++rf)
-#pragma unroll
-            for (int nf = 0; nf < NFW; ++nf) acc[h][rf][nf] *= p.w_inv;
-    float* stat = reinterpret_cast<float*>(smem + 2 * STAGE);
-    float mean[RFW], rstd[RFW];
-#pragma unroll
-    for (int rf = 0; rf < RFW; ++rf) {
-        float s = 0.f;
-#pragma unroll
-        for (int h = 0; h < NH; ++h)
-#pragma unroll
-            for (int nf = 0; nf < NFW; ++nf) {
-                const f32x4 v = acc[h][rf][nf];
-                s += (v[0] + v[1]) + (v[2] + v[3]);
-            }
-        s += __shfl_xor(s, 16);
-        s += __shfl_xor(s, 32);
-        if (f_kg == 0) stat[cw * BM + rw * (16 * RFW) + rf * 16 + f_row] = s;
-    }
-    __syncthreads();
-#pragma unroll
-    for (int rf = 0; rf < RFW; ++rf) {
-        const int r = rw * (16 * RFW) + rf * 16 + f_row;
-        float sm = 0.f;
-#pragma unroll
-        for (int c = 0; c < CW; ++c) sm += stat[c * BM + r];
-        mean[rf] = sm * (1.0f / BN);
-        float q = 0.f;
-#pragma unroll
-        for (int h = 0; h < NH; ++h)
-#pragma unroll
-            for (int nf = 0; nf < NFW; ++nf)
-#pragma unroll
-                for (int j = 0; j < 4; ++j) {
-                    const float d = acc[h][rf][nf][j] - mean[rf];
-                    q = __builtin_fmaf(d, d, q);
-                }
-        q += __shfl_xor(q, 16);
-        q += __shfl_xor(q, 32);
-        if (f_kg == 0) stat[(CW + cw) * BM + r] = q;
-    }
-    __syncthreads();
-#pragma unroll
-    for (int rf = 0; rf < RFW; ++rf) {
-        const int r = rw * (16 * RFW) + rf * 16 + f_row;
-        float var = 0.f;
-#pragma unroll
-        for (int c = 0; c < CW; ++c) var += stat[(CW + c) * BM + r];
-        rstd[rf] = 1.0f / sqrtf(var * (1.0f / BN) + p.eps);
-    }
-#pragma unroll
-    for (int h = 0; h < NH; ++h)
-#pragma unroll
-        for (int nf = 0; nf < NFW; ++nf) {
-            const int n = h * BNH + cw * (16 * NFW) + nf * 16 + f_kg * 4;
-            const f32x4 g = *reinterpret_cast<const f32x4*>(p.gamma + n), b = *reinterpret_cast<const f32x4*>(p.beta + n);
-#pragma unroll
-            for (int rf = 0; rf < RFW; ++rf) {
-                if (!valid(rf)) continue;
-                const f32x4 v = acc[h][rf][nf];
-                const size_t off = xrow(rf) + n;
-                *reinterpret_cast<f32x4*>(p.x_out + off) = v;
-                f32x4 hv;
-#pragma unroll
-                for (int j = 0; j < 4; ++j) hv[j] = (v[j] - mean[rf]) * rstd[rf] * g[j] + b[j];
-                if (p.h_bf16 == 2) {
-                    split_store4(p.h_out, off, hv);
-                } else if (p.h_bf16) {
-                    const bf16x4 ho = {(__bf16)hv[0], (__bf16)hv[1], (__bf16)hv[2], (__bf16)hv[3]};
-                    *reinterpret_cast<bf16x4*>(reinterpret_cast<__bf16*>(p.h_out) + off) = ho;
-                } else {
-                    *reinterpret_cast<f32x4*>(reinterpret_cast<float*>(p.h_out) + off) = hv;
-                }
-            }
-        }
+    constexpr int PE = (int)sizeof(T) * 0;
+#include "pp_gemm_ln_body.h"
+}
+
+template <int PE>
+__global__ __launch_bounds__(C384::THREADS, C384::MINW) void patch_embed_ln_kernel(const PatchParams p) {
+    using T = std::conditional_t<(PE > 0), SplitH, float>;
+    using C = std::conditional_t<(PE > 0), C384, C768>;
+#include "pp_gemm_ln_body.h"
+}
+
+template <int PE>
+static int launch_patch(const PatchParams& p, hipStream_t s) {
+    auto kern = patch_embed_ln_kernel<PE>;
+    PP_HIP_CHECK(hipFuncSetAttribute(reinterpret_cast<const void*>(kern), hipFuncAttributeMaxDynamicSharedMemorySize, C384::LDS));
+    hipLaunchKernelGGL(kern, dim3(p.M / C384::BM), dim3(C384::THREADS), C384::LDS, s, p);
+    PP_LAUNCH_CHECK_AS("patch_embed_ln");
+    return PP_OK;
 }
 
 template <typename T, typename C>
@@ -341,3 +170,55 @@
     if (prec == PP_PREC_F16X3) return wide ? rl::launch<SplitH, rl::C768>(p, s) : rl::launch<SplitH, rl::C384>(p, s);
     return wide ? rl::launch<float, rl::C768>(p, s) : rl::launch<float, rl::C384>(p, s);
 }
+
+
+static const char* patch_embed_refusal(int prec, int img_is_f32, int M, int N, int K, int H, int W, int patch, int pad) {
+    if (prec != PP_PREC_F16X3) return "pp_patch_embed_layernorm: split-fp16 operands only";
+    if (img_is_f32) return "pp_patch_embed_layernorm: uint8 crops only (an already preprocessed fp32 input takes pp_preproc_im2col + pp_gemm_residual_layernorm)";
+    if (N != pp::rl::C384::BN) return "pp_patch_embed_layernorm: built for an embedding width of 384";
+    if (patch != 16 || K != 3 * 16 * 16) return "pp_patch_embed_layernorm: patch size must be 16 (K = 768)";
+    if (M <= 0 || M % pp::rl::C384::BM != 0) return "pp_patch_embed_layernorm: the token rows must be a multiple of 96";
+    if (H <= 0 || W <= 0 || W % 4 != 0 || pad < 0 || H + 2 * pad < 16 || W + 2 * pad < 16) return "pp_patch_embed_layernorm: the crop width must be a multiple of 4";
+    return nullptr;
+}
+
+extern "C" int pp_patch_embed_layernorm_supported(int prec, int img_is_f32, int M, int N, int K, int H, int W, int patch, int pad) {
+    return pp::option("patch_embed_fused") != 0 && patch_embed_refusal(prec, img_is_f32, M, N, K, H, W, patch, pad) == nullptr;
+}
+
+extern "C" int pp_patch_embed_layernorm_ws(const void* img, int img_is_f32, int B, int passes, int H, int W, int patch, int pad,
+                                           const float* mean_host, const float* std_host, int bgr_to_rgb, int prec, const void* weight,
+                                           const float* bias, const float* residual, int res_mod, float* x_out, const float* gamma,
+                                           const float* beta, float eps, void* h_out, int h_bf16, int M, int N, int K, int ldw,
+                                           float w_inv_scale, void* stream) {
+    using namespace pp;
+    {
+        unsigned u;
+        __builtin_memcpy(&u, &w_inv_scale, 4);
+        PP_REQUIRE((u >> 31) == 0 && (u & 0x007fffffu) == 0 && ((u >> 23) & 0xffu) >= 127 - 40 && ((u >> 23) & 0xffu) <= 127 + 40, PP_ERR_INVALID_ARG,
+                   "pp_patch_embed_layernorm: the weight scale must be a power of two in [2^-40, 2^40]");
+    }
+    PP_REQUIRE(img && weight && x_out && gamma && beta && h_out, PP_ERR_INVALID_ARG, "pp_patch_embed_layernorm: NULL argument");
+    PP_REQUIRE(img_is_f32 || (mean_host && std_host), PP_ERR_INVALID_ARG, "pp_patch_embed_layernorm: mean/std are required for uint8 input");
+    PP_REQUIRE(passes == 1 || passes == 2, PP_ERR_INVALID_ARG, "pp_patch_embed_layernorm: passes must be 1 or 2");
+    PP_REQUIRE(B > 0 && H > 0 && W > 0 && pad >= 0 && M > 0 && K > 0, PP_ERR_INVALID_ARG, "pp_patch_embed_layernorm: bad shape");
+    if (const char* why = patch_embed_refusal(prec, img_is_f32, M, N, K, H, W, patch, pad)) return fail(PP_ERR_UNSUPPORTED, why);
+    const int Hp = (H + 2 * pad - patch) / patch + 1, Wp = (W + 2 * pad - patch) / patch + 1;
+    PP_REQUIRE((long long)passes * B * Hp * Wp == M, PP_ERR_INVALID_ARG, "pp_patch_embed_layernorm: M must be passes * B * patches per crop");
+    PP_REQUIRE(h_bf16 == PP_OUT_F32 || h_bf16 == PP_OUT_SPLIT, PP_ERR_UNSUPPORTED, "pp_patch_embed_layernorm: h_out is fp32 or the split-fp16 operand format");
+    PP_REQUIRE(ldw % 32 == 0 && ldw >= K, PP_ERR_UNSUPPORTED, "pp_patch_embed_layernorm: the weights' row pitch must be a multiple of 32 elements");
+    PP_REQUIRE((reinterpret_cast<uintptr_t>(img) & 3) == 0, PP_ERR_UNSUPPORTED, "pp_patch_embed_layernorm: the crops must be 4-byte aligned");
+    const size_t ib = (size_t)B * 3 * H * W, wb = ((size_t)(N - 1) * ldw + K) * 4;
+    PP_REQUIRE(ib < rl::OOB_OFFSET && wb < rl::OOB_OFFSET, PP_ERR_UNSUPPORTED, "pp_patch_embed_layernorm: operands must be smaller than 2 GiB");
+    rl::PatchParams p{};
+    p.A = nullptr; p.W = weight; p.bias = bias; p.residual = residual; p.x_out = x_out; p.h_out = h_out;
+    p.gamma = gamma; p.beta = beta; p.M = M; p.K = K; p.lda = K; p.ldw = ldw; p.res_mod = res_mod;
+    p.h_bf16 = h_bf16; p.a_bytes = 0; p.w_bytes = (unsigned)wb; p.eps = eps;
+    p.w_inv = w_inv_scale; p.w_s = 1.0f / w_inv_scale;
+    p.img = reinterpret_cast<const unsigned char*>(img); p.img_bytes = (unsigned)ib;
+    p.B = B; p.IH = H; p.IW = W; p.Wp = Wp; p.Np = Hp * Wp; p.pad = pad; p.bgr_to_rgb = bgr_to_rgb;
+    p.m0 = mean_host[0]; p.m1 = mean_host[1]; p.m2 = mean_host[2];
+    p.s0 = std_host[0]; p.s1 = std_host[1]; p.s2 = std_host[2];
+    hipStream_t s = reinterpret_cast<hipStream_t>(stream);
+    return option("patch_embed_fused") == 2 ? rl::launch_patch<64>(p, s) : rl::launch_patch<4>(p, s);
+}
diff --git a/probpose_code_amd/csrc/pp_gemm_ln_body.h b/probpose_code_amd/csrc/pp_gemm_ln_body.h
--- /dev/null
+++ b/probpose_code_amd/csrc/pp_gemm_ln_body.h
@@ -0,0 +1,334 @@
+    constexpr int BK = Prec<T>::BK;
+    constexpr int ESZ = (int)sizeof(T);
+    constexpr int BM = C::BM, BN = C::BN, NH = C::NH, RW = C::RW, CW = C::CW, RFW = C::RFW, NFW = C::NFW;
+    constexpr int STAGE = C::STAGE, W_TILE = C::W_TILE;
+    constexpr int DMA_PER_STAGE = PE ? BNH / 8 : C::DMA_PER_STAGE;
+    constexpr int DPW = (DMA_PER_STAGE + C::WAVES - 1) / C::WAVES;
+    static_assert(!PE || (__is_same(T, SplitH) && BM == 96 && NH == 1 && (PE == 4 || PE == 64)), "patch-embedding form");
+    extern __shared__ __attribute__((aligned(16))) char smem[];
+    const int tid = threadIdx.x, lane = tid & 63;
+    const int wv = __builtin_amdgcn_readfirstlane(tid >> 6);
+    const int rw = wv % RW, cw = wv / RW;
+    const int f_row = lane & 15, f_kg = lane >> 4;
+    const int m0 = blockIdx.x * BM;
+
+    const void* a_ptr;
+    unsigned a_len;
+    if constexpr (PE) {
+        a_ptr = pe_params<PE>(p).img;
+        a_len = pe_params<PE>(p).img_bytes;
+    } else {
+        a_ptr = p.A;
+        a_len = p.a_bytes;
+    }
+    const __amdgpu_buffer_rsrc_t a_rsrc = __builtin_amdgcn_make_buffer_rsrc(const_cast<void*>(a_ptr), 0, a_len, 0x00020000);
+    const __amdgpu_buffer_rsrc_t w_rsrc =
+        __builtin_amdgcn_make_buffer_rsrc(const_cast<void*>(p.W), 0, p.w_bytes, 0x00020000);
+    const int d_row = lane >> 3;
+    const unsigned d_chunk_bytes = (unsigned)(((lane & 7) ^ d_row) << 4);
+    unsigned s_voff[DPW];
+#pragma unroll
+    for (int j = 0; j < DPW; ++j) {
+        const int q = wv * DPW + j;
+        if (q < BNH / 8) {
+            const int n = q * 8 + d_row;
+            s_voff[j] = (unsigned)n * (unsigned)(p.ldw * ESZ) + d_chunk_bytes;
+        } else {
+            const int m = m0 + (q - BNH / 8) * 8 + d_row;
+            s_voff[j] = (q < DMA_PER_STAGE && m < p.M) ? (unsigned)m * (unsigned)(p.lda * ESZ) + d_chunk_bytes : OOB_OFFSET;
+        }
+    }
+    const unsigned half_bytes = (unsigned)BNH * (unsigned)(p.ldw * ESZ);
+    auto stage = [&](int half, int kt, int buf) {
+        char* dst = smem + buf * STAGE + wv * DPW * 1024;
+        const unsigned kb = (unsigned)(kt * BK * ESZ);
+#pragma unroll
+        for (int j = 0; j < DPW; ++j) {
+            const int q = wv * DPW + j;
+            if (q >= DMA_PER_STAGE) continue;
+            const unsigned vo = s_voff[j] == OOB_OFFSET ? OOB_OFFSET : s_voff[j] + kb;
+            if (q < BNH / 8)
+                __builtin_amdgcn_raw_ptr_buffer_load_lds(w_rsrc, (lds_ptr_t)(dst + j * 1024), 16, vo + (unsigned)half * half_bytes, 0, 0, 0);
+            else if constexpr (!PE)
+                __builtin_amdgcn_raw_ptr_buffer_load_lds(a_rsrc, (lds_ptr_t)(dst + j * 1024), 16, vo, 0, 0, 0);
+        }
+    };
+
+    constexpr int NPX = PE == 4 ? 4 : 16, NQ = NPX / 4, NDW = NQ + 1;
+    [[maybe_unused]] bool pe_on = false, pe_flip = false;
+    [[maybe_unused]] int pe_r = 0, pe_i = 0, pe_q = 0, pe_y0 = 0, pe_off = 0, pe_sh = 0, pe_dw = 0;
+    [[maybe_unused]] unsigned pe_mask[NPX / 2], pe_w[NDW];
+    if constexpr (PE) {
+        const auto& g = pe_params<PE>(p);
+        if constexpr (PE == 4) {
+            static_assert(PE != 4 || C::THREADS == 4 * PE_ITEMS, "four pixels per thread");
+            pe_on = true;
+            pe_r = tid >> 3;
+            pe_i = (tid >> 2) & 1;
+            pe_q = tid & 3;
+        } else {
+            pe_on = wv * 64 < PE_ITEMS;
+            pe_r = (tid >> 1) % BM;
+            pe_i = tid & 1;
+        }
+        const int m = m0 + pe_r;
+        const int pb = m / g.Np, tk = m - pb * g.Np;
+        const int pass = pb / g.B, b = pb - pass * g.B;
+        const int py = tk / g.Wp, px = tk - py * g.Wp;
+        const int x0 = 16 * px - g.pad;
+        const int lo = pass ? g.IW - 16 - x0 : x0;
+        const int a = (lo & ~3) + 4 * (pass ? NQ * (3 - pe_q) : NQ * pe_q) * (PE == 4);
+        pe_flip = pass != 0;
+        pe_sh = lo & 3;
+        pe_y0 = 16 * py - g.pad;
+        pe_off = (b * 3 * g.IH + pe_y0 + pe_i) * g.IW + a;
+#pragma unroll
+        for (int q = 0; q < NDW; ++q) pe_dw |= (a + 4 * q >= 0 && a + 4 * q + 4 <= g.IW) ? 1 << q : 0;
+#pragma unroll
+        for (int q = 0; q < NPX / 2; ++q) {
+            const int xa = x0 + NPX * pe_q + 2 * q, xb = xa + 1;
+            pe_mask[q] = ((xa >= 0 && xa < g.IW) ? 0x0000ffffu : 0u) | ((xb >= 0 && xb < g.IW) ? 0xffff0000u : 0u);
+        }
+    }
+    auto pe_load = [&](int kk) {
+        if constexpr (PE) {
+            const auto& g = pe_params<PE>(p);
+            const int c = kk >> 3, sc = g.bgr_to_rgb ? 2 - c : c;
+            const int y = pe_y0 + ((kk & 7) << 1) + pe_i;
+            const bool yok = y >= 0 && y < g.IH;
+            const int off = pe_off + (sc * g.IH + ((kk & 7) << 1)) * g.IW;
+            if (pe_on) {
+#pragma unroll
+                for (int q = 0; q < NDW; ++q) {
+                    unsigned vo = (yok && ((pe_dw >> q) & 1)) ? (unsigned)(off + 4 * q) : OOB_OFFSET;
+                    asm("" : "+v"(vo));
+                    pe_w[q] = __builtin_amdgcn_raw_buffer_load_b32(a_rsrc, vo, 0, 0);
+                }
+            }
+        }
+    };
+    auto pe_build = [&](int kk, int buf) {
+        if constexpr (PE) {
+            const auto& g = pe_params<PE>(p);
+            const int c = kk >> 3;
+            const float mean = c == 0 ? g.m0 : (c == 1 ? g.m1 : g.m2);
+            const float stdv = c == 0 ? g.s0 : (c == 1 ? g.s1 : g.s2);
+            const int y = pe_y0 + ((kk & 7) << 1) + pe_i;
+            const bool yok = y >= 0 && y < g.IH;
+            if (pe_on) {
+                unsigned t[NQ], d[NQ];
+#pragma unroll
+                for (int q = 0; q < NQ; ++q) t[q] = __builtin_amdgcn_alignbyte(pe_w[q + 1], pe_w[q], (unsigned)pe_sh);
+                const unsigned sel = pe_flip ? 0x00010203u : 0x03020100u;
+#pragma unroll
+                for (int q = 0; q < NQ; ++q) {
+                    const unsigned sq = pe_flip ? t[NQ - 1 - q] : t[q];
+                    d[q] = __builtin_amdgcn_perm(sq, sq, sel);
+                }
+                _Float16 hh[NPX], ll[NPX];
+#pragma unroll
+                for (int j = 0; j < NPX; ++j) {
+                    const float u = (float)((d[j >> 2] >> ((j & 3) * 8)) & 0xffu);
+                    const float v = (u - mean) / stdv;
+                    hh[j] = split_hi(v);
+                    ll[j] = split_lo(v, hh[j]);
+                }
+                char* arow = smem + buf * STAGE + W_TILE + pe_r * ROW_BYTES;
+                if constexpr (PE == 4) {
+                    typedef unsigned u32x2 __attribute__((ext_vector_type(2)));
+                    const u32x2 k = {yok ? pe_mask[0] : 0u, yok ? pe_mask[1] : 0u};
+                    const f16x4 h = {hh[0], hh[1], hh[2], hh[3]}, l = {ll[0], ll[1], ll[2], ll[3]};
+                    const int pos = (((2 * pe_i + (pe_q >> 1)) ^ (pe_r & 7)) << 4) + ((pe_q & 1) << 3);
+                    *reinterpret_cast<u32x2*>(arow + pos) = __builtin_bit_cast(u32x2, h) & k;
+                    *reinterpret_cast<u32x2*>(arow + (pos ^ 64)) = __builtin_bit_cast(u32x2, l) & k;
+                } else {
+                    f16x8 h0, h1, l0, l1;
+#pragma unroll
+                    for (int j = 0; j < 8; ++j) {
+                        h0[j] = hh[j];
+                        l0[j] = ll[j];
+                        h1[j] = hh[8 + j];
+                        l1[j] = ll[8 + j];
+                    }
+                    u32x4 k0, k1;
+#pragma unroll
+                    for (int q = 0; q < 4; ++q) {
+                        k0[q] = yok ? pe_mask[q] : 0u;
+                        k1[q] = yok ? pe_mask[4 + q] : 0u;
+                    }
+                    const int c0 = (2 * pe_i) ^ (pe_r & 7);
+                    *reinterpret_cast<u32x4*>(arow + (c0 << 4)) = __builtin_bit_cast(u32x4, h0) & k0;
+                    *reinterpret_cast<u32x4*>(arow + ((c0 ^ 1) << 4)) = __builtin_bit_cast(u32x4, h1) & k1;
+                    *reinterpret_cast<u32x4*>(arow + ((c0 ^ 4) << 4)) = __builtin_bit_cast(u32x4, l0) & k0;
+                    *reinterpret_cast<u32x4*>(arow + ((c0 ^ 5) << 4)) = __builtin_bit_cast(u32x4, l1) & k1;
+                }
+            }
+        }
+    };
+
+    const int nk = p.K / BK;
+    const int k_rot = (int)(blockIdx.x >> 3) % nk;
+    auto kstep = [&](int i) { const int k = i + k_rot; return k >= nk ? k - nk : k; };
+    pe_load(kstep(0));
+    stage(0, kstep(0), 0);
+    if constexpr (PE) {
+        pe_build(kstep(0), 0);
+        pe_load(kstep(1));
+    }
+
+    const int m_lane = m0 + rw * (16 * RFW) + f_row;
+    auto valid = [&](int rf) { return m_lane + rf * 16 < p.M; };
+    auto xrow = [&](int rf) { return (size_t)(m_lane + rf * 16) * BN; };
+    f32x4 acc[NH][RFW][NFW];
+#pragma unroll
+    for (int rf = 0; rf < RFW; ++rf) {
+        const int m = m_lane + rf * 16;
+        const size_t rrow = p.res_mod > 0 ? (size_t)(m % p.res_mod) * BN : xrow(rf);
+#pragma unroll
+        for (int h = 0; h < NH; ++h)
+#pragma unroll
+            for (int nf = 0; nf < NFW; ++nf) {
+                const int n = h * BNH + cw * (16 * NFW) + nf * 16 + f_kg * 4;
+                f32x4 v = {0.f, 0.f, 0.f, 0.f};
+                if (p.bias) v = *reinterpret_cast<const f32x4*>(p.bias + n);
+                if (p.residual && valid(rf)) v += *reinterpret_cast<const f32x4*>(p.residual + rrow + n);
+                acc[h][rf][nf] = v * p.w_s;
+            }
+    }
+    __syncthreads();
+#pragma unroll
+    for (int h = 0; h < NH; ++h) {
+        for (int kt = 0; kt < nk; ++kt) {
+            const int buf = (h * nk + kt) & 1;
+            if (kt + 1 < nk) stage(h, kstep(kt + 1), buf ^ 1);
+            else if (h + 1 < NH) stage(h + 1, kstep(0), buf ^ 1);
+            if constexpr (PE) {
+                if (kt + 1 < nk) pe_build(kstep(kt + 1), buf ^ 1);
+                if (kt + 2 < nk) pe_load(kstep(kt + 2));
+            }
+            const char* wbase = smem + buf * STAGE;
+            const char* abase = wbase + W_TILE;
+            if constexpr (__is_same(T, SplitH) && (RFW > NFW)) {
+                f16x8 fwh[NFW], fwl[NFW];
+#pragma unroll
+                for (int nf = 0; nf < NFW; ++nf) {
+                    fwh[nf] = *reinterpret_cast<const f16x8*>(wbase + swz(cw * (16 * NFW) + nf * 16 + f_row, f_kg));
+                    fwl[nf] = *reinterpret_cast<const f16x8*>(wbase + swz(cw * (16 * NFW) + nf * 16 + f_row, 4 + f_kg));
+                }
+#pragma unroll
+                for (int rf = 0; rf < RFW; ++rf) {
+                    const f16x8 fah = *reinterpret_cast<const f16x8*>(abase + swz(rw * (16 * RFW) + rf * 16 + f_row, f_kg));
+                    const f16x8 fal = *reinterpret_cast<const f16x8*>(abase + swz(rw * (16 * RFW) + rf * 16 + f_row, 4 + f_kg));
+#pragma unroll
+                    for (int nf = 0; nf < NFW; ++nf) acc[h][rf][nf] = split_mma(fwh[nf], fwl[nf], fah, fal, acc[h][rf][nf]);
+                }
+            } else if constexpr (__is_same(T, SplitH)) {
+                f16x8 fah[RFW], fal[RFW];
+#pragma unroll
+                for (int rf = 0; rf < RFW; ++rf) {
+                    fah[rf] = *reinterpret_cast<const f16x8*>(abase + swz(rw * (16 * RFW) + rf * 16 + f_row, f_kg));
+                    fal[rf] = *reinterpret_cast<const f16x8*>(abase + swz(rw * (16 * RFW) + rf * 16 + f_row, 4 + f_kg));
+                }
+#pragma unroll
+                for (int nf = 0; nf < NFW; ++nf) {
+                    const f16x8 fwh = *reinterpret_cast<const f16x8*>(wbase + swz(cw * (16 * NFW) + nf * 16 + f_row, f_kg));
+                    const f16x8 fwl = *reinterpret_cast<const f16x8*>(wbase + swz(cw * (16 * NFW) + nf * 16 + f_row, 4 + f_kg));
+#pragma unroll
+                    for (int rf = 0; rf < RFW; ++rf) acc[h][rf][nf] = split_mma(fwh, fwl, fah[rf], fal[rf], acc[h][rf][nf]);
+                }
+            } else {
+#pragma unroll
+                for (int ks = 0; ks < 2; ++ks) {
+                    u32x4 fa[RFW];
+#pragma unroll
+                    for (int rf = 0; rf < RFW; ++rf) fa[rf] = *reinterpret_cast<const u32x4*>(abase + swz(rw * (16 * RFW) + rf * 16 + f_row, ks * 4 + f_kg));
+#pragma unroll
+                    for (int nf = 0; nf < NFW; ++nf) {
+                        const u32x4 fw = *reinterpret_cast<const u32x4*>(wbase + swz(cw * (16 * NFW) + nf * 16 + f_row, ks * 4 + f_kg));
+#pragma unroll
+                        for (int rf = 0; rf < RFW; ++rf) acc[h][rf][nf] = mma(fw, fa[rf], acc[h][rf][nf], T{});
+                    }
+                }
+            }
+            __syncthreads();
+        }
+    }
+
+#pragma unroll
+    for (int h = 0; h < NH; ++h)
+#pragma unroll
+        for (int rf = 0; rf < RFW; ++rf)
+#pragma unroll
+            for (int nf = 0; nf < NFW; ++nf) acc[h][rf][nf] *= p.w_inv;
+    float* stat = reinterpret_cast<float*>(smem + 2 * STAGE);
+    float mean[RFW], rstd[RFW];
+#pragma unroll
+    for (int rf = 0; rf < RFW; ++rf) {
+        float s = 0.f;
+#pragma unroll
+        for (int h = 0; h < NH; ++h)
+#pragma unroll
+            for (int nf = 0; nf < NFW; ++nf) {
+                const f32x4 v = acc[h][rf][nf];
+                s += (v[0] + v[1]) + (v[2] + v[3]);
+            }
+        s += __shfl_xor(s, 16);
+        s += __shfl_xor(s, 32);
+        if (f_kg == 0) stat[cw * BM + rw * (16 * RFW) + rf * 16 + f_row] = s;
+    }
+    __syncthreads();
+#pragma unroll
+    for (int rf = 0; rf < RFW; ++rf) {
+        const int r = rw * (16 * RFW) + rf * 16 + f_row;
+        float sm = 0.f;
+#pragma unroll
+        for (int c = 0; c < CW; ++c) sm += stat[c * BM + r];
+        mean[rf] = sm * (1.0f / BN);
+        float q = 0.f;
+#pragma unroll
+        for (int h = 0; h < NH; ++h)
+#pragma unroll
+            for (int nf = 0; nf < NFW; ++nf)
+#pragma unroll
+                for (int j = 0; j < 4; ++j) {
+                    const float d = acc[h][rf][nf][j] - mean[rf];
+                    q = __builtin_fmaf(d, d, q);
+                }
+        q += __shfl_xor(q, 16);
+        q += __shfl_xor(q, 32);
+        if (f_kg == 0) stat[(CW + cw) * BM + r] = q;
+    }
+    __syncthreads();
+#pragma unroll
+    for (int rf = 0; rf < RFW; ++rf) {
+        const int r = rw * (16 * RFW) + rf * 16 + f_row;
+        float var = 0.f;
+#pragma unroll
+        for (int c = 0; c < CW; ++c) var += stat[(CW + c) * BM + r];
+        rstd[rf] = 1.0f / sqrtf(var * (1.0f / BN) + p.eps);
+    }
+#pragma unroll
+    for (int h = 0; h < NH; ++h)
+#pragma unroll
+        for (int nf = 0; nf < NFW; ++nf) {
+            const int n = h * BNH + cw * (16 * NFW) + nf * 16 + f_kg * 4;
+            const f32x4 g = *reinterpret_cast<const f32x4*>(p.gamma + n), b = *reinterpret_cast<const f32x4*>(p.beta + n);
+#pragma unroll
+            for (int rf = 0; rf < RFW; ++rf) {
+                if (!valid(rf)) continue;
+                const f32x4 v = acc[h][rf][nf];
+                const size_t off = xrow(rf) + n;
+                *reinterpret_cast<f32x4*>(p.x_out + off) = v;
+                f32x4 hv;
+#pragma unroll
+                for (int j = 0; j < 4; ++j) hv[j] = (v[j] - mean[rf]) * rstd[rf] * g[j] + b[j];
+                if (p.h_bf16 == 2) {
+                    split_store4(p.h_out, off, hv);
+                } else if (p.h_bf16) {
+                    const bf16x4 ho = {(__bf16)hv[0], (__bf16)hv[1], (__bf16)hv[2], (__bf16)hv[3]};
+                    *reinterpret_cast<bf16x4*>(reinterpret_cast<__bf16*>(p.h_out) + off) = ho;
+                } else {
+                    *reinterpret_cast<f32x4*>(reinterpret_cast<float*>(p.h_out) + off) = hv;
+                }
+            }
+        }
diff --git a/probpose_code_amd/engine.py b/probpose_code_amd/engine.py
--- a/probpose_code_amd/engine.py
+++ b/probpose_code_amd/engine.py
@@ -237,7 +237,7 @@
         small = self._small_at(M)
         fused_layer = self.precision == "f16x3" and self.fuse_qkv_attn and bool(self._proj_packed) and not small
         ws = dict(
-            patches=buf("patches", (M, 3 * self.P * self.P)), x=buf("x", (M, E), f32), h=buf("h", (M, E)),
+            patches=None if self._patch_fused_at(M) else buf("patches", (M, 3 * self.P * self.P)), x=buf("x", (M, E), f32), h=buf("h", (M, E)),
             feat=buf("feat", (M, E)), logits=buf("logits", (nb, self.K, self.Hh * self.Wh), f32),
             qkv=None if (fused_layer or (small and self.fuse_qkv_attn)) else buf("qkv", (M, 3 * E)),
             qkv2=None if (fused_layer or small) else buf("qkv", (M, 3 * E)),
@@ -277,6 +277,20 @@
         return bool(self.small_plan and M < self.small_rows_below and self.E % 64 == 0 and self.w.ffn_dims % 64 == 0 and self.E <= 1024
                     and self.w.has("l0.fc1.w") and self.w.has("l0.proj.w") and (3 * self.P * self.P) % 64 == 0)
 
+    def _patch_fused_at(self, M: int, img_is_f32: bool = False) -> bool:
+        return bool(self.precision == "f16x3" and self.fuse_resln and not self._small_at(M)
+                    and _lib.lib.pp_patch_embed_layernorm_supported(self.prec, int(img_is_f32), int(M), self.E, 3 * self.P * self.P, self.H, self.W,
+                                                                    self.P, self.pad))
+
+    def _patches(self, ws, M: int) -> torch.Tensor:
+        if ws["patches"] is None:
+            shape = _lib.PlanShape(prec=self.prec, n_img=M // self.Np, n_tokens=self.Np, embed=self.E, ffn=self.w.ffn_dims, patch_k=3 * self.P * self.P,
+                                   n_keypoints=self.K, feat_h=self.Hp, feat_w=self.Wp, heat_h=self.Hh, heat_w=self.Wh,
+                                   deconv_channels=self.w.deconv_channels[0] if self.w.deconv_channels else 0)
+            nbytes = _lib.workspace_bytes("patches", shape)
+            ws["patches"] = torch.empty(nbytes, dtype=torch.uint8, device=self.device).view(self.dtype).view(M, 3 * self.P * self.P)
+        return ws["patches"]
+
     def _ln_fold_at(self, M: int) -> bool:
         return (self.ln_fold and _lib.get_option("linear_dma") != 0
                 and _lib.lib.pp_linear_ln_folded_supported(int(M), self.E, self.E, 1) == 2
@@ -317,10 +331,19 @@
         M = B * passes * self.Np
         E, Fd, w = self.E, self.w.ffn_dims, self.w
         ob = self.fmt
-        self._call("im2col", "pp_preproc_im2col", self.prec, imgs_u8.data_ptr(), int(imgs_u8.dtype == torch.float32),
-                  ws["patches"].data_ptr(), B, passes, self.H, self.W, self.P, self.pad, self.mean.ctypes.data,
-                  self.std.ctypes.data, int(self.bgr_to_rgb), st)
         Kp = 3 * self.P * self.P
+        is_f32 = imgs_u8.dtype == torch.float32
+        if imgs_u8.data_ptr() % 4 == 0 and self._patch_fused_at(M, is_f32):
+            self._call("patch_embed_ln", "pp_patch_embed_layernorm_ws", imgs_u8.data_ptr(), 0, B, passes, self.H, self.W, self.P, self.pad,
+                       self.mean.ctypes.data, self.std.ctypes.data, int(self.bgr_to_rgb), self.prec, w["patch_w"].data_ptr(), w["patch_b"].data_ptr(),
+                       w["pos_embed"].data_ptr(), self.Np, ws["x"].data_ptr(), w["l0.ln1.w"].data_ptr(), w["l0.ln1.b"].data_ptr(), self.ln_eps,
+                       ws["h"].data_ptr(), self.fmt, M, E, Kp, Kp, float(w.inv("patch_w")), st)
+            patch_done = True
+        else:
+            patch_done = False
+            self._call("im2col", "pp_preproc_im2col", self.prec, imgs_u8.data_ptr(), int(is_f32),
+                       self._patches(ws, M).data_ptr(), B, passes, self.H, self.W, self.P, self.pad, self.mean.ctypes.data,
+                       self.std.ctypes.data, int(self.bgr_to_rgb), st)
         scale = self.hd ** -0.5
         fused = self.fuse_resln and (E == 384 or (E == 768 and self._resln_768))
         L = w.num_layers
@@ -338,8 +361,9 @@
 
         if self._small_at(M):
             return self._layers_small(ws, st, B * passes, M)
-        res_ln(ws["patches"], w["patch_w"], w["patch_b"], Kp, w["l0.ln1.w"], w["l0.ln1.b"], ws["h"],
-               residual=w["pos_embed"], res_mod=self.Np)
+        if not patch_done:
+            res_ln(ws["patches"], w["patch_w"], w["patch_b"], Kp, w["l0.ln1.w"], w["l0.ln1.b"], ws["h"],
+                   residual=w["pos_embed"], res_mod=self.Np)
         if self._ln_fold_at(M):
             return self._layers_ln_folded(ws, st, B * passes, M)
         qkv_done = False
```

Result: no change. 15040 crops/s (median of 6 runs) (+0.4%).
